# ootts/EasyHeC

Measured on AMD Instinct MI355X. Metric: mask-render fwd+bwd frames/sec, xArm7 50k-tri @1280x720x8-view, higher is better.
Workload: dtype f32; 1 GPU; xarm7_1280x720_8view; robot=xarm7 (41096 tris, 20525 verts), views_per_gpu=8, global_views=8, links=8, antialias=True, optimizer=Adam lr 3e-3 wd 5e-4, ref_sums=bound once, mask_output=False, step=HIP launch chain, parallelism=single GPU

## Files before the change

### easyhec_amd/_lib.py

```python
import ctypes
import os

_HERE = os.path.dirname(os.path.abspath(__file__))
LIB_PATH = os.environ.get("EHR_LIB") or os.path.join(_HERE, "libehr_hip.so")
_lib = None

c_void_p, c_int, c_size_t, c_float = ctypes.c_void_p, ctypes.c_int, ctypes.c_size_t, ctypes.c_float

SIGNATURES = {
    "ehr_version": (c_int, []),
    "ehr_last_error": (ctypes.c_char_p, []),
    "ehr_device_count": (c_int, []),
    "ehr_device_arch": (ctypes.c_char_p, [c_int]),
    "ehr_ctx_create": (c_int, [c_int, ctypes.POINTER(c_void_p)]),
    "ehr_ctx_destroy": (c_int, [c_void_p]),
    "ehr_ctx_scratch_bytes": (c_size_t, [c_void_p]),
    "ehr_tile_flags_bytes": (c_size_t, [c_int, c_int, c_int]),
    "ehr_rasterize_fwd": (c_int, [c_void_p, c_void_p, c_void_p, c_void_p, c_int, c_int, c_int, c_int, c_int, c_void_p,
                                  c_void_p, c_void_p, c_void_p]),
    "ehr_rasterize_grad": (c_int, [c_void_p, c_void_p, c_void_p, c_void_p, c_int, c_int, c_int, c_int, c_int, c_int,
                                   c_void_p, c_void_p, c_void_p]),
    "ehr_rasterize_grad_db": (c_int, [c_void_p, c_void_p, c_void_p, c_void_p, c_int, c_int, c_int, c_int, c_int, c_int,
                                   c_void_p, c_void_p]),
    "ehr_interpolate_fwd": (c_int, [c_void_p, c_void_p, c_void_p, c_int, c_int, c_int, c_int, c_int, c_int, c_int,
                                    c_void_p, c_void_p, c_void_p]),
    "ehr_interpolate_grad": (c_int, [c_void_p, c_void_p, c_void_p, c_void_p, c_int, c_int, c_int, c_int, c_int, c_int,
                                     c_int, c_void_p, c_void_p, c_void_p, c_void_p]),
    "ehr_interpolate_da_fwd": (c_int, [c_void_p, c_void_p, c_void_p, c_void_p, c_void_p] + [c_int] * 8 + [c_void_p, c_void_p]),
    "ehr_interpolate_da_grad": (c_int, [c_void_p, c_void_p, c_void_p, c_void_p, c_void_p, c_void_p] + [c_int] * 8 +
                                [c_void_p, c_void_p, c_void_p]),
    "ehr_topology_scratch_bytes": (c_size_t, [c_int]),
    "ehr_antialias_topology": (c_int, [c_void_p, c_int, c_void_p, c_void_p, c_size_t, c_void_p]),
    "ehr_antialias_work_bytes": (c_size_t, [c_int, c_int, c_int]),
    "ehr_antialias_fwd": (c_int, [c_void_p, c_void_p, c_void_p, c_void_p, c_void_p, c_int, c_int, c_int, c_int, c_int,
                                  c_int, c_int, c_void_p, c_void_p, c_void_p, c_void_p]),
    "ehr_antialias_fwd_zg": (c_int, [c_void_p, c_void_p, c_void_p, c_void_p, c_void_p, c_int, c_int, c_int, c_int, c_int,
                                     c_int, c_int, c_void_p, c_void_p, c_void_p, c_void_p, c_void_p]),
    "ehr_antialias_grad": (c_int, [c_void_p, c_void_p, c_void_p, c_void_p, c_void_p, c_void_p, c_int, c_int, c_int,
                                   c_int, c_int, c_int, c_int, c_void_p, c_void_p, c_void_p]),
    "ehr_fused_plan": (c_int, [c_void_p, c_int, c_int, c_int, c_int, c_int, c_int, c_float, c_void_p, c_void_p,
                                c_void_p, c_void_p]),
    "ehr_render_mask_loss": (c_int, [c_void_p, c_void_p, c_void_p, c_void_p, c_void_p, c_void_p, c_void_p, c_void_p,
                                     c_int, c_int, c_int, c_int, c_int, c_int, c_void_p, c_void_p, c_void_p,
                                     c_void_p]),
    "ehr_fused_status": (c_int, [c_void_p]),
    "ehr_fused_bind_ref": (c_int, [c_void_p, c_void_p, c_void_p]),
    "ehr_pose_forward": (c_int, [c_void_p, c_void_p, c_void_p, c_int, c_int, c_int, c_int, c_float, c_float, c_void_p,
                                 c_void_p, c_void_p, c_void_p, c_int, c_void_p]),
    "ehr_pose_backward": (c_int, [c_void_p, c_void_p, c_void_p, c_void_p, c_void_p, c_int, c_int, c_int, c_int,
                                  c_float, c_float, c_void_p, c_void_p]),
    "ehr_pose_adam": (c_int, [c_void_p, c_void_p, c_void_p, c_void_p, c_void_p, c_float, c_float, c_float, c_float,
                              c_float, c_void_p, c_void_p, c_void_p]),
    "ehr_solver_step": (c_int, [c_void_p] * 9 + [c_int] * 6 + [c_float] * 2 + [c_void_p] * 5 + [c_int, c_void_p] +
                        [c_float] * 5 + [c_void_p] * 8 + [c_int, c_void_p]),
    "ehr_solver_step_multi": (c_int, [c_void_p] * 9 + [c_int] * 7 + [c_float] * 2 + [c_void_p] * 5 + [c_int, c_void_p] +
                              [c_float] * 5 + [c_void_p] * 8 + [c_void_p]),
    "ehr_fused_bind_ref_shared": (c_int, [c_void_p, c_void_p, c_int, c_void_p]),
    "ehr_fused_bind_weight": (c_int, [c_void_p, c_void_p, c_int, c_void_p]),
    "ehr_mask_variance": (c_int, [c_void_p] * 5 + [c_int] * 7 + [c_void_p, c_void_p, c_int, c_void_p]),
    "ehr_mask_overlap": (c_int, [c_void_p] * 6 + [c_int] * 7 + [c_void_p, c_void_p, c_int, c_void_p]),
    "ehr_comm_unique_id": (c_int, [c_void_p]),
    "ehr_comm_init": (c_int, [c_void_p, c_void_p, c_int, c_int]),
    "ehr_comm_allreduce": (c_int, [c_void_p, c_void_p, c_int, c_void_p]),
    "ehr_comm_destroy": (c_int, [c_void_p]),
    "ehr_comm_p2p_export": (c_int, [c_void_p, c_void_p]),
    "ehr_comm_p2p_open": (c_int, [c_void_p, c_void_p, c_int, c_int]),
    "ehr_comm_p2p_step": (c_int, [c_void_p] * 6 + [c_float] * 5 + [c_void_p, c_void_p, c_void_p]),
    "ehr_comm_p2p_close": (c_int, [c_void_p]),
    "ehr_graph_begin": (c_int, [c_void_p, ctypes.POINTER(c_void_p)]),
    "ehr_graph_end": (c_int, [c_void_p]),
    "ehr_graph_launch": (c_int, [c_void_p, c_void_p]),
    "ehr_graph_release": (c_int, [c_void_p]),
    "ehr_fused_timing": (c_int, [c_void_p, c_int]),
    "ehr_fused_timing_read": (c_int, [c_void_p, ctypes.POINTER(c_float), ctypes.POINTER(c_int)]),
    "ehr_joint_forward": (c_int, [c_void_p] * 6 + [c_int] * 3 + [c_void_p, c_void_p, c_int, c_void_p, c_void_p, c_void_p]),
    "ehr_joint_backward_adam": (c_int, [c_void_p] * 3 + [c_int] * 5 + [c_float] * 2 + [c_void_p] * 10 + [c_float] * 5 +
                                [c_void_p, c_void_p]),
}


def lib():
    global _lib
    if _lib is None:
        if not os.path.exists(LIB_PATH):
            raise RuntimeError(
                f"{LIB_PATH} is missing: build it with `python -m easyhec_amd.build` (hipcc --offload-arch=gfx950). "
                "easyhec_amd has no CPU or PyTorch fallback for the render path.")
        l = ctypes.CDLL(LIB_PATH)
        for name, (res, args) in SIGNATURES.items():
            fn = getattr(l, name)
            fn.restype = res
            fn.argtypes = args
        _lib = l
    return _lib


def has_multistart():
    if not os.path.exists(LIB_PATH):
        return False
    return hasattr(_lib if _lib is not None else ctypes.CDLL(LIB_PATH), "ehr_solver_step_multi")


def has_pose_search():
    if not os.path.exists(LIB_PATH):
        return False
    return hasattr(_lib if _lib is not None else ctypes.CDLL(LIB_PATH), "ehr_mask_overlap")


def has_weighted_loss():
    if not os.path.exists(LIB_PATH):
        return False
    return hasattr(_lib if _lib is not None else ctypes.CDLL(LIB_PATH), "ehr_fused_bind_weight")


def has_joint_offsets():
    if not os.path.exists(LIB_PATH):
        return False
    l = _lib if _lib is not None else ctypes.CDLL(LIB_PATH)
    return hasattr(l, "ehr_joint_forward") and hasattr(l, "ehr_joint_backward_adam")


EHR_ERR_OVERFLOW = -3
EHR_ERR_RETRY = -4


def check(rc, what):
    if rc != 0:
        msg = lib().ehr_last_error().decode("utf-8", "replace")
        raise RuntimeError(f"{what}: {msg} (code {rc})")


def ptr(t):
    return None if t is None else c_void_p(t.data_ptr())
```

### easyhec_amd/csrc/ehr_device.h

```cpp
#pragma once
#include <hip/hip_runtime.h>
#include <stdint.h>

#define EHR_TILE_W 32
#define EHR_TILE_H 8
#define EHR_TILE_THREADS 256

namespace ehr {

typedef long long i64;
typedef unsigned long long u64;

__device__ __forceinline__ float tri_to_float(int x) {
    return (x <= 0x01000000) ? (float)x : __int_as_float(0x4a800000 + x);
}
__device__ __forceinline__ int float_to_tri(float f) {
    return (f <= 16777216.f) ? (int)f : (__float_as_int(f) - 0x4a800000);
}
__device__ __forceinline__ unsigned ord_key(float f) {
    unsigned u = __float_as_uint(f);
    return (u & 0x80000000u) ? ~u : (u | 0x80000000u);
}
__device__ __forceinline__ float ord_unkey(unsigned k) {
    unsigned u = (k & 0x80000000u) ? (k & 0x7fffffffu) : ~k;
    return __uint_as_float(u);
}
__device__ __forceinline__ float sat01(float x) { return x > 0.f ? (x < 1.f ? x : 1.f) : 0.f; }
__device__ __forceinline__ bool same_sign(float a, float b) {
    return (int)(__float_as_uint(a) ^ __float_as_uint(b)) >= 0;
}

__device__ __forceinline__ int snap_coord(float v, float w, float scale) {
    float s = v / w;
    float t = s * scale;
    t = fmaxf(fminf(t, 1073741824.f), -1073741824.f);
    return (int)rintf(t);
}

__device__ __forceinline__ float4 transform_vertex(const float* __restrict__ M, float x, float y, float z) {
    float4 o;
    o.x = fmaf(M[0], x, fmaf(M[1], y, fmaf(M[2], z, M[3])));
    o.y = fmaf(M[4], x, fmaf(M[5], y, fmaf(M[6], z, M[7])));
    o.z = fmaf(M[8], x, fmaf(M[9], y, fmaf(M[10], z, M[11])));
    o.w = fmaf(M[12], x, fmaf(M[13], y, fmaf(M[14], z, M[15])));
    return o;
}

struct ClipPoly {
    float4 q0, q1, q2, q3;
    int n;
};

__device__ __forceinline__ float4 clip_lerp(const float4& a, const float4& b, float da, float db) {
    float t = da / (da - db);
    float4 r;
    r.x = a.x + t * (b.x - a.x);
    r.y = a.y + t * (b.y - a.y);
    r.z = a.z + t * (b.z - a.z);
    r.w = a.w + t * (b.w - a.w);
    return r;
}

__device__ __forceinline__ ClipPoly clip_near_poly(const float4 p[3]) {
    ClipPoly c;
    c.n = 0;
    c.q0 = c.q1 = c.q2 = c.q3 = make_float4(0.f, 0.f, 0.f, 0.f);
    float d0 = p[0].z + p[0].w, d1 = p[1].z + p[1].w, d2 = p[2].z + p[2].w;
    bool all_in = (p[0].w > 0.f) && (p[1].w > 0.f) && (p[2].w > 0.f) && (d0 >= 0.f) && (d1 >= 0.f) && (d2 >= 0.f);
    if (all_in) {
        c.q0 = p[0];
        c.q1 = p[1];
        c.q2 = p[2];
        c.n = 3;
        return c;
    }
    const int mask = (d0 >= 0.f ? 1 : 0) | (d1 >= 0.f ? 2 : 0) | (d2 >= 0.f ? 4 : 0);
    const float4 I0 = clip_lerp(p[0], p[1], d0, d1);
    const float4 I1 = clip_lerp(p[1], p[2], d1, d2);
    const float4 I2 = clip_lerp(p[2], p[0], d2, d0);
    switch (mask) {
        case 1: c.q0 = p[0]; c.q1 = I0; c.q2 = I2; c.n = 3; break;
        case 2: c.q0 = I0; c.q1 = p[1]; c.q2 = I1; c.n = 3; break;
        case 4: c.q0 = I1; c.q1 = p[2]; c.q2 = I2; c.n = 3; break;
        case 3: c.q0 = p[0]; c.q1 = p[1]; c.q2 = I1; c.q3 = I2; c.n = 4; break;
        case 6: c.q0 = I0; c.q1 = p[1]; c.q2 = p[2]; c.q3 = I2; c.n = 4; break;
        case 5: c.q0 = p[0]; c.q1 = I0; c.q2 = I1; c.q3 = p[2]; c.n = 4; break;
        case 7: c.q0 = p[0]; c.q1 = p[1]; c.q2 = p[2]; c.n = 3; break;
        default: c.n = 0; break;
    }
    if (c.n < 3) c.n = 0;
    bool ok = (c.q0.w > 0.f) && (c.q1.w > 0.f) && (c.q2.w > 0.f) && (c.n < 4 || c.q3.w > 0.f);
    if (!ok) c.n = 0;
    return c;
}

struct Coverage {
    int X[3], Y[3];
    int ix0, ix1, iy0, iy1;
    bool valid;
};

__device__ __forceinline__ Coverage setup_coverage(const float4& a, const float4& b, const float4& c, int W, int H) {
    Coverage cv;
    const float sx = (float)(W * 8), sy = (float)(H * 8);
    cv.X[0] = snap_coord(a.x, a.w, sx);
    cv.Y[0] = snap_coord(a.y, a.w, sy);
    cv.X[1] = snap_coord(b.x, b.w, sx);
    cv.Y[1] = snap_coord(b.y, b.w, sy);
    cv.X[2] = snap_coord(c.x, c.w, sx);
    cv.Y[2] = snap_coord(c.y, c.w, sy);
    i64 area2 = (i64)(cv.X[1] - (i64)cv.X[0]) * (i64)(cv.Y[2] - (i64)cv.Y[0]) -
                (i64)(cv.X[2] - (i64)cv.X[0]) * (i64)(cv.Y[1] - (i64)cv.Y[0]);
    cv.valid = area2 != 0;
    if (area2 < 0) {
        int tx = cv.X[1], ty = cv.Y[1];
        cv.X[1] = cv.X[2];
        cv.Y[1] = cv.Y[2];
        cv.X[2] = tx;
        cv.Y[2] = ty;
    }
    int xmin = min(cv.X[0], min(cv.X[1], cv.X[2])), xmax = max(cv.X[0], max(cv.X[1], cv.X[2]));
    int ymin = min(cv.Y[0], min(cv.Y[1], cv.Y[2])), ymax = max(cv.Y[0], max(cv.Y[1], cv.Y[2]));
    const int cx = 8 - 8 * W, cy = 8 - 8 * H;
    int ix0 = (xmin - cx + 15) >> 4, ix1 = (xmax - cx) >> 4;
    int iy0 = (ymin - cy + 15) >> 4, iy1 = (ymax - cy) >> 4;
    ix0 = max(ix0, 0);
    iy0 = max(iy0, 0);
    ix1 = min(ix1, W - 1);
    iy1 = min(iy1, H - 1);
    cv.ix0 = ix0;
    cv.ix1 = ix1;
    cv.iy0 = iy0;
    cv.iy1 = iy1;
    if (ix0 > ix1 || iy0 > iy1) cv.valid = false;
    return cv;
}

struct EdgeEval {
    i64 e[3];
    i64 sx[3], sy[3];
};

__device__ __forceinline__ EdgeEval setup_edges(const Coverage& cv, int ix, int iy, int W, int H) {
    EdgeEval ee;
    const i64 cx = 8 - 8 * (i64)W, cy = 8 - 8 * (i64)H;
    i64 Px = 16 * (i64)ix + cx, Py = 16 * (i64)iy + cy;
#pragma unroll
    for (int k = 0; k < 3; k++) {
        int j = (k == 2) ? 0 : k + 1;
        i64 dX = (i64)cv.X[j] - cv.X[k], dY = (i64)cv.Y[j] - cv.Y[k];
        bool tl = (dY < 0) || (dY == 0 && dX < 0);
        ee.e[k] = dX * (Py - cv.Y[k]) - dY * (Px - cv.X[k]) - (tl ? 0 : 1);
        ee.sx[k] = -16 * dY;
        ee.sy[k] = 16 * dX;
    }
    return ee;
}

__device__ __forceinline__ void eval_pixel(const float4 p[3], float fx, float fy, float& a0, float& a1, float& a2) {
    float p0x = p[0].x - fx * p[0].w, p0y = p[0].y - fy * p[0].w;
    float p1x = p[1].x - fx * p[1].w, p1y = p[1].y - fy * p[1].w;
    float p2x = p[2].x - fx * p[2].w, p2y = p[2].y - fy * p[2].w;
    a0 = p1x * p2y - p1y * p2x;
    a1 = p2x * p0y - p2y * p0x;
    a2 = p0x * p1y - p0y * p1x;
}

__device__ __forceinline__ float eval_zw(const float4 p[3], float a0, float a1, float a2) {
    float z = (p[0].z * a0 + p[1].z * a1) + p[2].z * a2;
    float w = (p[0].w * a0 + p[1].w * a1) + p[2].w * a2;
    return z / w;
}


__device__ __forceinline__ bool rational_gt(float n0, float n1, float d0, float d1) {
    float l = n0 * d1, r = n1 * d0;
    bool flip = (d0 < 0.f) != (d1 < 0.f);
    return flip ? (l < r) : (l > r);
}

__device__ __forceinline__ int max_idx3(float n0, float n1, float n2, float d0, float d1, float d2) {
    bool g10 = rational_gt(n1, n0, d1, d0);
    bool g20 = rational_gt(n2, n0, d2, d0);
    bool g21 = rational_gt(n2, n1, d2, d1);
    if (g20 && g21) return 2;
    if (g10) return 1;
    return 0;
}

struct AAPair {
    bool found;
    int di;
    int tri1;
    float alpha;
};

__device__ __forceinline__ AAPair aa_analyze(const float4 p[3], const float4 o[3], int px, int py, int d, bool chose0,
                                             int W, int H) {
    AAPair r;
    r.found = false;
    r.di = 0;
    r.tri1 = chose0 ? 0 : 1;
    r.alpha = 0.f;
    float xh = .5f * (float)W, yh = .5f * (float)H;
    float w0 = 1.f / p[0].w, w1 = 1.f / p[1].w, w2 = 1.f / p[2].w;
    float ow0 = 1.f / o[0].w, ow1 = 1.f / o[1].w, ow2 = 1.f / o[2].w;
    float fx = (float)px + .5f - xh;
    float fy = (float)py + .5f - yh;
    float x0 = p[0].x * w0 * xh - fx, y0 = p[0].y * w0 * yh - fy;
    float x1 = p[1].x * w1 * xh - fx, y1 = p[1].y * w1 * yh - fy;
    float x2 = p[2].x * w2 * xh - fx, y2 = p[2].y * w2 * yh - fy;
    float ox0 = o[0].x * ow0 * xh - fx, oy0 = o[0].y * ow0 * yh - fy;
    float ox1 = o[1].x * ow1 * xh - fx, oy1 = o[1].y * ow1 * yh - fy;
    float ox2 = o[2].x * ow2 * xh - fx, oy2 = o[2].y * ow2 * yh - fy;

    float bb = (x1 - x0) * (y2 - y0) - (x2 - x0) * (y1 - y0);
    float a0 = (x1 - ox0) * (y2 - oy0) - (x2 - ox0) * (y1 - oy0);
    float a1 = (x2 - ox1) * (y0 - oy1) - (x0 - ox1) * (y2 - oy1);
    float a2 = (x0 - ox2) * (y1 - oy2) - (x1 - ox2) * (y0 - oy2);
    bool s0 = same_sign(a0, bb), s1 = same_sign(a1, bb), s2 = same_sign(a2, bb);
    if (!(s0 || s1 || s2)) return r;

    if (d) {
        float s;
        s = x0; x0 = y0; y0 = s;
        s = x1; x1 = y1; y1 = s;
        s = x2; x2 = y2; y2 = s;
    }
    float dx0 = x2 - x1, dx1 = x0 - x2, dx2 = x1 - x0;
    float dy0 = y2 - y1, dy1 = y0 - y2, dy2 = y1 - y0;
    const float F32_MAX = 3.402823466e+38f;
    float dc = -F32_MAX;
    float ds = chose0 ? 1.f : -1.f;
    float d0 = ds * (x1 * dy0 - y1 * dx0);
    float d1 = ds * (x2 * dy1 - y2 * dx1);
    float d2 = ds * (x0 * dy2 - y0 * dx2);
    if (same_sign(y1, y2)) { d0 = -F32_MAX; dy0 = 1.f; }
    if (same_sign(y2, y0)) { d1 = -F32_MAX; dy1 = 1.f; }
    if (same_sign(y0, y1)) { d2 = -F32_MAX; dy2 = 1.f; }
    int di = max_idx3(d0, d1, d2, dy0, dy1, dy2);
    if (di == 0 && s0 && fabsf(dy0) >= fabsf(dx0)) dc = d0 / dy0;
    if (di == 1 && s1 && fabsf(dy1) >= fabsf(dx1)) dc = d1 / dy1;
    if (di == 2 && s2 && fabsf(dy2) >= fabsf(dx2)) dc = d2 / dy2;
    const float eps = .0625f;
    if (dc > -eps && dc < 1.f + eps) {
        dc = fminf(fmaxf(dc, 0.f), 1.f);
        r.found = true;
        r.di = di;
        r.alpha = ds * (.5f - dc);
    }
    return r;
}

__device__ __forceinline__ void aa_pos_grad(float4 p1, float4 p2, int px, int py, int d, float alpha, float dd, int W,
                                            int H, float g1[3], float g2[3]) {
    float pxh = .5f * (float)W, pyh = .5f * (float)H;
    float fx = (float)px + .5f - pxh;
    float fy = (float)py + .5f - pyh;
    if (d) {
        float s;
        s = p1.x; p1.x = p1.y; p1.y = s;
        s = p2.x; p2.x = p2.y; p2.y = s;
        s = pxh; pxh = pyh; pyh = s;
        s = fx; fx = fy; fy = s;
    }
    float w1 = 1.f / p1.w, w2 = 1.f / p2.w;
    float x1 = p1.x * w1 * pxh - fx, y1 = p1.y * w1 * pyh - fy;
    float x2 = p2.x * w2 * pxh - fx, y2 = p2.y * w2 * pyh - fy;
    float dx = x2 - x1, dy = y2 - y1;
    float db = x1 * dy - y1 * dx;
    float ep = copysignf(1e-3f, dy);
    float iy = 1.f / (dy + ep);
    float dby = db * iy;
    float iw1 = -w1 * iy * dd;
    float iw2 = w2 * iy * dd;
    float gp1x = iw1 * pxh * y2;
    float gp2x = iw2 * pxh * y1;
    float gp1y = iw1 * pyh * (dby - x2);
    float gp2y = iw2 * pyh * (dby - x1);
    float gp1w = -(p1.x * gp1x + p1.y * gp1y) * w1;
    float gp2w = -(p2.x * gp2x + p2.y * gp2y) * w2;
    if (d) {
        float s;
        s = gp1x; gp1x = gp1y; gp1y = s;
        s = gp2x; gp2x = gp2y; gp2y = s;
    }
    if (fabsf(alpha) >= 0.5f) {
        gp1x = gp1y = gp1w = 0.f;
        gp2x = gp2y = gp2w = 0.f;
    }
    g1[0] = gp1x; g1[1] = gp1y; g1[2] = gp1w;
    g2[0] = gp2x; g2[1] = gp2y; g2[2] = gp2w;
}

constexpr int EHR_FLAG_TW = 32, EHR_FLAG_TH = 8;
__host__ __device__ __forceinline__ int flag_ntx(int W) { return (W + EHR_FLAG_TW - 1) / EHR_FLAG_TW; }
__host__ __device__ __forceinline__ int flag_nty(int H) { return (H + EHR_FLAG_TH - 1) / EHR_FLAG_TH; }
__device__ __forceinline__ bool tile_occupied(const unsigned char* __restrict__ flags, int b, int ix, int iy, int W, int H) {
    if (!flags) return true;
    const int ntx = flag_ntx(W), nty = flag_nty(H);
    return flags[((size_t)b * nty + (iy / EHR_FLAG_TH)) * ntx + (ix / EHR_FLAG_TW)] != 0;
}


__device__ __forceinline__ int lane_id() { return __lane_id(); }

template <int K>
__device__ __forceinline__ unsigned wave_xor_u32(unsigned v) {
    const int iv = (int)v;
    if (K == 1) return (unsigned)__builtin_amdgcn_update_dpp(iv, iv, 0xB1, 0xf, 0xf, false);
    if (K == 2) return (unsigned)__builtin_amdgcn_update_dpp(iv, iv, 0x4E, 0xf, 0xf, false);
    if (K == 4) {
        const int up = __builtin_amdgcn_update_dpp(iv, iv, 0x104, 0xf, 0xf, false);
        const int dn = __builtin_amdgcn_update_dpp(iv, iv, 0x114, 0xf, 0xf, false);
        return (unsigned)((__lane_id() & 4) ? dn : up);
    }
    if (K == 8) return (unsigned)__builtin_amdgcn_update_dpp(iv, iv, 0x128, 0xf, 0xf, false);
    if (K == 16) {
        const auto r = __builtin_amdgcn_permlane16_swap(v, v, false, false);
        return (__lane_id() & 16) ? r[0] : r[1];
    }
    const auto r = __builtin_amdgcn_permlane32_swap(v, v, false, false);
    return (__lane_id() & 32) ? r[0] : r[1];
}
template <int K>
__device__ __forceinline__ float wave_xor(float v) { return __uint_as_float(wave_xor_u32<K>(__float_as_uint(v))); }
template <int K>
__device__ __forceinline__ int wave_xor(int v) { return (int)wave_xor_u32<K>((unsigned)v); }
template <int K>
__device__ __forceinline__ long long wave_xor(long long v) {
    const unsigned long long u = (unsigned long long)v;
    const unsigned lo = wave_xor_u32<K>((unsigned)u), hi = wave_xor_u32<K>((unsigned)(u >> 32));
    return (long long)((unsigned long long)lo | ((unsigned long long)hi << 32));
}
template <int K>
__device__ __forceinline__ double wave_xor(double v) {
    const unsigned long long u = (unsigned long long)__double_as_longlong(v);
    const unsigned lo = wave_xor_u32<K>((unsigned)u), hi = wave_xor_u32<K>((unsigned)(u >> 32));
    return __longlong_as_double((long long)((unsigned long long)lo | ((unsigned long long)hi << 32)));
}

__device__ __forceinline__ float wave_sum(float v) {
    v += wave_xor<32>(v);
    v += wave_xor<16>(v);
    v += wave_xor<8>(v);
    v += wave_xor<4>(v);
    v += wave_xor<2>(v);
    v += wave_xor<1>(v);
    return v;
}

__device__ __forceinline__ int wave_sum12_element(int lane) {
    return 6 * ((lane >> 5) & 1) + 3 * ((lane >> 4) & 1) + ((lane & 8) ? 2 : ((lane >> 2) & 1));
}
__device__ __forceinline__ float wave_sum12(const float v[12], int lane) {
    const bool b32 = lane & 32, b16 = lane & 16, b8 = lane & 8, b4 = lane & 4;
    float a[6];
#pragma unroll
    for (int i = 0; i < 6; i++) {
        const float keep = b32 ? v[6 + i] : v[i], send = b32 ? v[i] : v[6 + i];
        a[i] = keep + wave_xor<32>(send);
    }
    float b[3];
#pragma unroll
    for (int i = 0; i < 3; i++) {
        const float keep = b16 ? a[3 + i] : a[i], send = b16 ? a[i] : a[3 + i];
        b[i] = keep + wave_xor<16>(send);
    }
    const float r0 = wave_xor<8>(b8 ? b[0] : b[2]);
    const float r1 = wave_xor<8>(b[1]);
    const float c0 = (b8 ? b[2] : b[0]) + r0, c1 = b[1] + r1;
    const float keep = b8 ? c0 : (b4 ? c1 : c0), send = b8 ? c0 : (b4 ? c0 : c1);
    float d = keep + wave_xor<4>(send);
    d += wave_xor<2>(d);
    d += wave_xor<1>(d);
    return d;
}

}
```

### easyhec_amd/csrc/ehr_fused.hip

```cpp
#include <stdlib.h>

#include <algorithm>

#include "ehr_fused_core.h"

namespace ehr {
constexpr int MAX_LINKS = 32;
}

using namespace ehr;

extern "C" {

int ehr_fused_plan(ehr_ctx* ctx, int B, int L, int V, int T, int H, int W, float slack, const float* verts,
                   const int32_t* tris, const int32_t* tri_link, const int32_t* opp) {
    if (!ctx) return fail(EHR_ERR_INVALID, "ehr_fused_plan: ctx is NULL");
    if (B <= 0 || L <= 0 || L > MAX_LINKS || V < 0 || T < 0 || H <= 0 || W <= 0 || H > 32768 || W > 32768)
        return fail(EHR_ERR_INVALID, "ehr_fused_plan: bad sizes (1 <= L <= %d)", MAX_LINKS);
    if (!(slack > 0.f)) slack = 0.f;
    if (ctx->gexec) {
        EHR_HIP(hipGraphExecDestroy(ctx->gexec));
        ctx->gexec = nullptr;
    }
    int rc0 = vbuf_plan(ctx, B, L, V, T, H, W, slack, verts, tris, tri_link, opp);
    if (rc0) return rc0;
    int dev = 0;
    EHR_HIP(hipGetDevice(&dev));
    hipDeviceProp_t prop;
    EHR_HIP(hipGetDeviceProperties(&prop, dev));
    ctx->num_cus = prop.multiProcessorCount;
    ctx->pB = B;
    ctx->pL = L;
    ctx->pV = V;
    ctx->pT = T;
    ctx->pH = H;
    ctx->pW = W;
    return EHR_OK;
}

static int fused_chain(ehr_ctx* ctx, const float* verts, const int32_t* tris, const int32_t* tri_link,
                       const int32_t* vert_link, const int32_t* opp, float* mvp, const float* ref, int B, int L, int V,
                       int T, int H, int W, float* mask, float* loss, float* grad_mvp, const StepHead* head,
                       const StepTail* tail, void* stream_, int multi_views = 0) {
    if (!ctx) return fail(EHR_ERR_INVALID, "fused op: ctx is NULL");
    if (!verts || !tris || !tri_link || !vert_link || !opp || !mvp || !ref || !loss)
        return fail(EHR_ERR_INVALID, "fused op: NULL tensor");
    if (ctx->pB != B || ctx->pL != L || ctx->pV != V || ctx->pT != T || ctx->pH != H || ctx->pW != W)
        return fail(EHR_ERR_INVALID, "fused op: shape differs from the planned one; call ehr_fused_plan first");
    return vbuf_chain(ctx, verts, tris, vert_link, opp, mvp, ref, B, L, V, T, H, W, mask, loss, grad_mvp, head,
                      tail, (hipStream_t)stream_, multi_views);
}

int ehr_render_mask_loss(ehr_ctx* ctx, const float* verts, const int32_t* tris, const int32_t* tri_link,
                         const int32_t* vert_link, const int32_t* opp, const float* mvp, const float* ref, int B,
                         int L, int V, int T, int H, int W, float* mask, float* loss, float* grad_mvp, void* stream) {
    return fused_chain(ctx, verts, tris, tri_link, vert_link, opp, const_cast<float*>(mvp), ref, B, L, V, T, H, W, mask,
                       loss, grad_mvp, nullptr, nullptr, stream);
}

static int step_head_tail(const char* who, ehr_ctx* ctx, ehr::Scratch ehr_ctx::*hstate, int nviews, int defer_adam,
                          int L, const float* K, const float* link_poses, float near_, float far_, float* dof, float* adam_m,
                          float* adam_v, int32_t* step, float* history, int history_rows, int32_t* history_row, float lr,
                          float beta1, float beta2, float eps, float weight_decay, float* tc_jac, const float* grad_mvp,
                          float* red, float* loss_out, float* grad_out, StepHead& head, StepTail& tail) {
    if (!ctx) return fail(EHR_ERR_INVALID, "%s: ctx is NULL", who);
    if (!K || !link_poses || !dof || !adam_m || !adam_v || !step || !tc_jac || !grad_mvp || !red)
        return fail(EHR_ERR_INVALID, "%s: NULL tensor", who);
    if (L > MAX_LINKS) return fail(EHR_ERR_INVALID, "%s: more than %d links", who, MAX_LINKS);
    if (history && !history_row) return fail(EHR_ERR_INVALID, "%s: history given without history_row", who);
    head.dof = dof;
    head.K = K;
    head.link_poses = link_poses;
    head.tc_jac = tc_jac;
    head.hist_row = history_row;
    head.history = history;
    head.history_rows = history_rows;
    head.n = near_;
    head.f = far_;
    head.adam_step = step;
    head.hstate = (int*)(ctx->*hstate).ptr;
    head.view0 = 0;
    head.nviews = nviews;
    tail.K = K;
    tail.link_poses = link_poses;
    tail.tc_jac = tc_jac;
    tail.red = red;
    tail.dof = dof;
    tail.m = adam_m;
    tail.v = adam_v;
    tail.step = step;
    tail.loss_out = loss_out;
    tail.grad_out = grad_out;
    tail.n = near_;
    tail.f = far_;
    tail.lr = lr;
    tail.b1 = beta1;
    tail.b2 = beta2;
    tail.eps = eps;
    tail.wd = weight_decay;
    tail.defer_adam = defer_adam;
    return EHR_OK;
}

int ehr_solver_step(ehr_ctx* ctx, const float* verts, const int32_t* tris, const int32_t* tri_link,
                    const int32_t* vert_link, const int32_t* opp, const float* K, const float* link_poses,
                    const float* ref, int B, int L, int V, int T, int H, int W, float near_, float far_, float* dof,
                    float* adam_m, float* adam_v, int32_t* step, float* history, int history_rows, int32_t* history_row,
                    float lr, float beta1,
                    float beta2, float eps, float weight_decay, float* mvp, float* tc_jac, float* mask, float* loss_b,
                    float* grad_mvp, float* red, float* loss_out, float* grad_out, int defer_adam, void* stream) {
    StepHead head;
    StepTail tail;
    int rc = step_head_tail("ehr_solver_step", ctx, &ehr_ctx::vb_hstate, B, defer_adam, L, K, link_poses, near_, far_, dof,
                            adam_m, adam_v, step, history, history_rows, history_row, lr, beta1, beta2, eps, weight_decay,
                            tc_jac, grad_mvp, red, loss_out, grad_out, head, tail);
    if (rc) return rc;
    return fused_chain(ctx, verts, tris, tri_link, vert_link, opp, mvp, ref, B, L, V, T, H, W, mask, loss_b, grad_mvp,
                       &head, &tail, stream);
}

int ehr_solver_step_multi(ehr_ctx* ctx, const float* verts, const int32_t* tris, const int32_t* tri_link,
                          const int32_t* vert_link, const int32_t* opp, const float* K, const float* link_poses,
                          const float* ref, int P, int Bv, int L, int V, int T, int H, int W, float near_, float far_,
                          float* dof, float* adam_m, float* adam_v, int32_t* step, float* history, int history_rows,
                          int32_t* history_row, float lr, float beta1, float beta2, float eps, float weight_decay,
                          float* mvp, float* tc_jac, float* mask, float* loss_b, float* grad_mvp, float* red,
                          float* loss_out, float* grad_out, void* stream) {
    StepHead head;
    StepTail tail;
    int rc = step_head_tail("ehr_solver_step_multi", ctx, &ehr_ctx::vb_hstate_m, Bv, 0, L, K, link_poses, near_, far_, dof,
                            adam_m, adam_v, step, history, history_rows, history_row, lr, beta1, beta2, eps, weight_decay,
                            tc_jac, grad_mvp, red, loss_out, grad_out, head, tail);
    if (rc) return rc;
    if (P <= 0 || Bv <= 0 || (long long)P * Bv > 0x7fffffffll / 64)
        return fail(EHR_ERR_INVALID, "ehr_solver_step_multi: bad P x Bv");
    if (ctx->pB != P * Bv || ctx->vb_hstate_m.cap < (size_t)VB_HSTATE_INTS * P * sizeof(int))
        return fail(EHR_ERR_INVALID, "ehr_solver_step_multi: call ehr_fused_plan for B = P x Bv = %d views first", P * Bv);
    return fused_chain(ctx, verts, tris, tri_link, vert_link, opp, mvp, ref, P * Bv, L, V, T, H, W, mask, loss_b, grad_mvp,
                       &head, &tail, stream, Bv);
}

int ehr_fused_bind_ref(ehr_ctx* ctx, const float* ref, void* stream) {
    return ehr_fused_bind_ref_shared(ctx, ref, ctx ? ctx->pB : 0, stream);
}

int ehr_fused_bind_ref_shared(ehr_ctx* ctx, const float* ref, int Bv, void* stream) {
    if (!ctx) return fail(EHR_ERR_INVALID, "ehr_fused_bind_ref: ctx is NULL");
    if (ctx->capturing) return fail(EHR_ERR_INVALID, "ehr_fused_bind_ref: not inside a graph capture");
    if (ctx->gexec) {
        EHR_HIP(hipGraphExecDestroy(ctx->gexec));
        ctx->gexec = nullptr;
    }
    if (!ref) {
        ctx->vb_ref = nullptr;
        return EHR_OK;
    }
    if (ctx->pB == 0) return fail(EHR_ERR_INVALID, "ehr_fused_bind_ref: call ehr_fused_plan first");
    return vbuf_bind_ref(ctx, ref, Bv, (hipStream_t)stream);
}

int ehr_fused_bind_weight(ehr_ctx* ctx, const float* weight, int Bv, void* stream) {
    (void)stream;
    if (!ctx) return fail(EHR_ERR_INVALID, "ehr_fused_bind_weight: ctx is NULL");
    if (ctx->capturing) return fail(EHR_ERR_INVALID, "ehr_fused_bind_weight: not inside a graph capture");
    if (weight) {
        if (ctx->pB == 0) return fail(EHR_ERR_INVALID, "ehr_fused_bind_weight: call ehr_fused_plan first");
        if (Bv <= 0 || ctx->pB % Bv != 0)
            return fail(EHR_ERR_INVALID, "ehr_fused_bind_weight: the plan's %d views are not a multiple of %d", ctx->pB, Bv);
    }
    if (ctx->gexec) {
        EHR_HIP(hipGraphExecDestroy(ctx->gexec));
        ctx->gexec = nullptr;
    }
    ctx->vb_ref = nullptr;
    ctx->vb_weight = weight;
    ctx->vb_weight_views = weight ? Bv : 0;
    return EHR_OK;
}

int ehr_fused_status(ehr_ctx* ctx) {
    if (!ctx) return fail(EHR_ERR_INVALID, "ehr_fused_status: ctx is NULL");
    if (ctx->pB == 0) return EHR_OK;
    if (!ctx->vb_acc.ptr) return EHR_OK;
    EHR_HIP(hipDeviceSynchronize());
    int m4[4] = {0, 0, 0, 0};
    int rc0 = vbuf_meta_read(ctx, m4);
    if (rc0) return rc0;
    if (m4[EHR_META_OVERFLOW] & VB_FLAG_NEED_SLOW) ctx->vb_slow_needed = true;
    if (m4[EHR_META_OVERFLOW] & ~VB_FLAG_NEED_SLOW)
        return fail(EHR_ERR_OVERFLOW, "fused path: an accumulator or the blended-pair spill pool overflowed");
    if (m4[EHR_META_OVERFLOW] & VB_FLAG_NEED_SLOW)
        return fail(EHR_ERR_RETRY, "fused path: the step met triangles for the general-triangle pass (near-plane clipping or "
                    "more than 512 pixels wide), which the solver step had not been launching; it is switched on now: run the "
                    "step again (its NaN left the optimiser state untouched; re-capture a captured chain)");
    return EHR_OK;
}


int ehr_graph_begin(ehr_ctx* ctx, void** capture_stream) {
    if (!ctx || !capture_stream) return fail(EHR_ERR_INVALID, "ehr_graph_begin: NULL argument");
    if (ctx->capturing) return fail(EHR_ERR_INVALID, "ehr_graph_begin: a capture is already open on this context");
    if (ctx->timing) return fail(EHR_ERR_INVALID, "ehr_graph_begin: disable ehr_fused_timing first");
    if (!ctx->cap_stream) EHR_HIP(hipStreamCreateWithFlags(&ctx->cap_stream, hipStreamNonBlocking));
    if (ctx->gexec) {
        EHR_HIP(hipGraphExecDestroy(ctx->gexec));
        ctx->gexec = nullptr;
    }
    EHR_HIP(hipStreamBeginCapture(ctx->cap_stream, hipStreamCaptureModeThreadLocal));
    ctx->capturing = true;
    *capture_stream = (void*)ctx->cap_stream;
    return EHR_OK;
}

int ehr_graph_end(ehr_ctx* ctx) {
    if (!ctx || !ctx->capturing) return fail(EHR_ERR_INVALID, "ehr_graph_end: no open capture");
    ctx->capturing = false;
    hipGraph_t graph = nullptr;
    EHR_HIP(hipStreamEndCapture(ctx->cap_stream, &graph));
    if (!graph) return fail(EHR_ERR_HIP, "ehr_graph_end: the capture was invalidated");
    hipError_t e = hipGraphInstantiate(&ctx->gexec, graph, nullptr, nullptr, 0);
    (void)hipGraphDestroy(graph);
    if (e != hipSuccess) {
        ctx->gexec = nullptr;
        return fail(EHR_ERR_HIP, "hipGraphInstantiate failed: %s", hipGetErrorString(e));
    }
    ctx->gexec_reallocs = ctx->scratch_moves();
    return EHR_OK;
}

int ehr_graph_launch(ehr_ctx* ctx, void* stream) {
    if (!ctx || !ctx->gexec) return fail(EHR_ERR_INVALID, "ehr_graph_launch: no instantiated graph");
    if (ctx->gexec_reallocs != ctx->scratch_moves())
        return fail(EHR_ERR_INVALID, "ehr_graph_launch: library scratch was reallocated after the capture; capture again");
    EHR_HIP(hipGraphLaunch(ctx->gexec, (hipStream_t)stream));
    return EHR_OK;
}

int ehr_graph_release(ehr_ctx* ctx) {
    if (!ctx) return EHR_OK;
    if (ctx->capturing) {
        hipGraph_t graph = nullptr;
        (void)hipStreamEndCapture(ctx->cap_stream, &graph);
        if (graph) (void)hipGraphDestroy(graph);
        ctx->capturing = false;
    }
    if (ctx->gexec) {
        EHR_HIP(hipGraphExecDestroy(ctx->gexec));
        ctx->gexec = nullptr;
    }
    return EHR_OK;
}

int ehr_fused_timing(ehr_ctx* ctx, int enable) {
    if (!ctx) return fail(EHR_ERR_INVALID, "ehr_fused_timing: ctx is NULL");
    ctx->timing = enable != 0;
    ctx->ev_used = 0;
    return EHR_OK;
}

int ehr_fused_timing_read(ehr_ctx* ctx, float* ms, int* ncalls) {
    if (!ctx || !ms || !ncalls) return fail(EHR_ERR_INVALID, "ehr_fused_timing_read: NULL argument");
    EHR_HIP(hipDeviceSynchronize());
    const size_t per = EHR_FUSED_STAGES + 1;
    const size_t n = ctx->ev_used / per;
    for (int s = 0; s < EHR_FUSED_STAGES; s++) ms[s] = 0.f;
    for (size_t c = 0; c < n; c++)
        for (int s = 0; s < EHR_FUSED_STAGES; s++) {
            float t = 0.f;
            EHR_HIP(hipEventElapsedTime(&t, ctx->ev[c * per + s], ctx->ev[c * per + s + 1]));
            ms[s] += t;
        }
    *ncalls = (int)n;
    ctx->ev_used = 0;
    return EHR_OK;
}

}
```

### easyhec_amd/csrc/ehr_host.h

```cpp
#pragma once
#include <hip/hip_runtime.h>
#include <stdint.h>
#include <stdio.h>

#include <string>
#include <vector>

#include "../../include/ehr.h"

struct ehr_ctx;

namespace ehr {

void set_error(const std::string& msg);
int fail(int code, const char* fmt, ...);

#define EHR_HIP(call)                                                                                   \
    do {                                                                                                \
        hipError_t e_ = (call);                                                                         \
        if (e_ != hipSuccess)                                                                           \
            return ::ehr::fail(EHR_ERR_HIP, "%s failed: %s (%s:%d)", #call, hipGetErrorString(e_), __FILE__, __LINE__); \
    } while (0)

#define EHR_LAUNCH_CHECK()                                                                              \
    do {                                                                                                \
        hipError_t e_ = hipGetLastError();                                                              \
        if (e_ != hipSuccess)                                                                           \
            return ::ehr::fail(EHR_ERR_HIP, "kernel launch failed: %s (%s:%d)", hipGetErrorString(e_), __FILE__, __LINE__); \
    } while (0)

struct Scratch {
    void* ptr = nullptr;
    size_t cap = 0;
    int reserve(size_t bytes);
    void release();
    unsigned long long moves = 0;
    bool pinned = false;
};

int zero_words(void* dst, size_t nwords, hipStream_t stream);
int fill_words(void* dst, size_t nwords, unsigned value, hipStream_t stream);
int copy_words(void* dst, const void* src, size_t nwords, hipStream_t stream);

struct StepHead;
struct StepTail;
struct RasterShape {
    int B, V, T, H, W, ranged;
    bool operator==(const RasterShape& o) const { return B == o.B && V == o.V && T == o.T && H == o.H && W == o.W && ranged == o.ranged; }
};
#define VB_LOSS_SLOTS 32
#define VB_LOSS_STRIDE 16
#define VB_FLAG_NEED_SLOW 4
#define VB_MAX_UNITS 512
#define VB_SPILL_ITEMS (1 << 20)
int vbuf_plan(ehr_ctx* ctx, int B, int L, int V, int T, int H, int W, float slack, const float* verts,
              const int32_t* tris, const int32_t* tri_link, const int32_t* opp);
int vbuf_meta_read(ehr_ctx* ctx, int* meta4);
int vbuf_bind_ref(ehr_ctx* ctx, const float* ref, int views, hipStream_t stream);
int vbuf_score(ehr_ctx* ctx, const float* verts, const int32_t* tris, const int32_t* vert_link, const float* mvp, int Q, int S,
               int L, int V, int T, int H, int W, long long* score, unsigned char* count, hipStream_t stream, int* handled);
int vbuf_overlap(ehr_ctx* ctx, const float* verts, const int32_t* tris, const int32_t* vert_link, const float* mvp,
                 const float* ref, int Q, int S, int L, int V, int T, int H, int W, long long* overlap, long long* ref_area,
                 hipStream_t stream, int* handled);
int vbuf_chain(ehr_ctx* ctx, const float* verts, const int32_t* tris, const int32_t* vert_link,
               const int32_t* opp, float* mvp, const float* ref, int B, int L, int V, int T, int H, int W, float* mask,
               float* loss, float* grad_mvp, const StepHead* head, const StepTail* tail, hipStream_t stream,
               int multi_views = 0);

}

struct ehr_ctx {
    int device = 0;
    ehr::Scratch counts;
    unsigned long long counts_clean = ~0ull;
    bool vb_slow_needed = false;
    ehr::Scratch ranges;
    std::vector<int32_t> ranges_last;
    unsigned long long ranges_moves = ~0ull;
    ehr::Scratch rkeys;
    unsigned long long rkeys_clean = ~0ull;
    ehr::Scratch offsets;
    ehr::Scratch entries;
    size_t entries_cap = 0;
    int* host_pinned = nullptr;
    hipEvent_t ev_size[2] = {nullptr, nullptr};
    bool size_valid[2] = {false, false};
    ehr::RasterShape size_shape[2] = {};
    int size_slot = 0;
    int pB = 0, pL = 0, pV = 0, pT = 0, pH = 0, pW = 0;
    int num_cus = 256;
    ehr::Scratch vb_clus;
    ehr::Scratch vb_heavy;
    ehr::Scratch vb_idx;
    const void* vb_plan_tris = nullptr;
    const void* vb_plan_opp = nullptr;
    const void* vb_plan_verts = nullptr;
    int vb_nc = 0;
    int vb_jcap = 0;
    int vb_chunk = 0;
    ehr::Scratch vb_boxes;
    ehr::Scratch vb_units;
    ehr::Scratch vb_acc;
    ehr::Scratch vb_posc;
    bool vb_lazy = false;
    ehr::Scratch vb_jobs;
    ehr::Scratch vb_spill;
    int vb_spill_cap = 0;
    ehr::Scratch vb_refsum;
    const float* vb_ref = nullptr;
    int vb_ref_views = 0;
    const float* vb_weight = nullptr;
    int vb_weight_views = 0;
    ehr::Scratch vb_hstate;
    ehr::Scratch vb_hstate_m;
    ehr::Scratch sc_counts, sc_offsets, sc_entries, sc_posc;
    ehr::Scratch sc_img;
    size_t sc_entries_cap = 0;
    ehr::Scratch sc_clus, sc_misc;
    int sc_nc = 0;
    const void* sc_key[3] = {nullptr, nullptr, nullptr};
    int sc_key_n[3] = {0, 0, 0};
    unsigned long long sc_hash = 0;
    bool sc_mixed = false;
    void* comm = nullptr;
    int comm_ranks = 0;
    void* p2p_mail = nullptr;
    void* p2p_peer[EHR_P2P_MAX_RANKS] = {};
    int p2p_ranks = 0, p2p_rank = 0;
    hipStream_t cap_stream = nullptr;
    hipGraphExec_t gexec = nullptr;
    unsigned long long gexec_reallocs = 0;
    unsigned long long scratch_moves() const {
        unsigned long long n = 0;
        for (const ehr::Scratch* s : {&counts, &offsets, &entries, &vb_clus, &vb_heavy, &vb_idx, &vb_boxes, &vb_units, &vb_acc,
                                      &vb_posc, &vb_jobs, &vb_spill, &vb_refsum, &vb_hstate, &vb_hstate_m, &sc_counts, &sc_offsets, &sc_entries, &sc_posc, &sc_clus, &sc_misc, &sc_img})
            n += s->moves;
        return n;
    }
    bool capturing = false;
    bool timing = false;
    std::vector<hipEvent_t> ev;
    size_t ev_used = 0;
};
```

### easyhec_amd/csrc/ehr_vbuf.hip

```cpp
#include <stdlib.h>
#include <string.h>

#include <algorithm>
#include <utility>
#include <vector>

#include "ehr_fused_core.h"

namespace ehr {

constexpr int VB_RW = EHR_TILE_W + 2;
constexpr int VB_RH = EHR_TILE_H + 2;
constexpr int VB_RN = VB_RW * VB_RH;
constexpr int VB_WORDS = (VB_RN + 63) / 64;
constexpr int VB_LBOX_STRIDE = 16;
constexpr int VB_HEAVY_T_DEFAULT = 3000;
constexpr int VB_HEAVY_CAP = 4096;
constexpr int VB_MED_CAP = 2048;
constexpr int VB_MED_T_DEFAULT = 1500;
constexpr int VB_PRIO_LONG = 3;
constexpr int VB_PRIO_HEAVY = 2;
constexpr int VB_JOB_ITEMS = 64;
constexpr int VB_SPILL_BLOCK = 2048;
constexpr u64 VB_EMPTY = ~0ull;
constexpr int VB_VERTEX_GRID = 5;
constexpr int VB_JOB_GRID = 4;
constexpr int VB_COMPOSITE_GRID = 6;
constexpr int VB_SCORE_COUNT_GRID = 4;
constexpr int VB_SLOW_GRID = 32;
constexpr bool VB_XCD_SPLIT = true;
constexpr int VB_FAST_EXTENT = 8192;

constexpr int VB_XCDS = 8;
constexpr int VB_XCD_BITS = __builtin_ctz(VB_XCDS);
static_assert(VB_XCDS == 1 << VB_XCD_BITS, "a workgroup finds its XCD with a mask and a shift");
__host__ __device__ constexpr int vb_xcd_share(int n) { return (n + VB_XCDS - 1) >> VB_XCD_BITS; }
__host__ __device__ constexpr int vb_xcd_round_up(int n) { return (n + VB_XCDS - 1) & ~(VB_XCDS - 1); }

enum VbLine {
    VB_LINE_JOB_CURSOR = 0,
    VB_LINE_COMP_ARRIVE = VB_LINE_JOB_CURSOR + VB_XCDS,
    VB_LINE_SLOW_COUNT = VB_LINE_COMP_ARRIVE + VB_XCDS,
    VB_LINES
};
__host__ __device__ __forceinline__ int* vb_line(int* meta, int k) {
    return (int*)((((uintptr_t)(meta + EHR_META_INTS)) + 127) & ~(uintptr_t)127) + 32 * k;
}
constexpr size_t VB_META_BYTES = EHR_META_INTS * sizeof(int) + (VB_LINES + 1) * 128;

#define VB_WAVE_SYNC() asm volatile("s_waitcnt lgkmcnt(0)" ::: "memory")

struct VbItem {
    int packed;
    int v1, v2;
    float alpha;
};

struct VbCarve {
    uintptr_t at;
    template <class T>
    T* take(size_t n, size_t align = alignof(T)) {
        at = (at + align - 1) & ~(uintptr_t)(align - 1);
        T* const p = (T*)at;
        at += n * sizeof(T);
        return p;
    }
};

struct VbSlots {
    float* jval;
    VbItem* jitems;
    int* jn;
    int* jspill;
    int* jbase;
    unsigned* jutile;
    int4* slow_list;
    int jcap;
};
constexpr size_t VB_SLOT_BYTES = 256 * sizeof(float) + VB_JOB_ITEMS * sizeof(VbItem) + 2 * sizeof(int) + sizeof(int4);
static_assert(VB_SLOT_BYTES == 1024 + 1024 + 8 + 16, "job slot: 2072 bytes");
static VbSlots vb_slots(void* base, size_t jcap, size_t units, size_t* bytes = nullptr) {
    VbCarve c{(uintptr_t)base};
    VbSlots s;
    s.jval = c.take<float>(jcap * 256);
    s.jitems = c.take<VbItem>(jcap * VB_JOB_ITEMS);
    s.jn = c.take<int>(jcap);
    s.jspill = c.take<int>(jcap);
    s.jbase = c.take<int>(units + 1);
    s.jutile = c.take<unsigned>(units);
    s.slow_list = c.take<int4>(jcap, 16);
    s.jcap = (int)jcap;
    if (bytes) *bytes = c.at - (uintptr_t)base;
    return s;
}

constexpr bool vb_interior(int i) {
    return (i % VB_RW) >= 1 && (i % VB_RW) <= EHR_TILE_W && (i / VB_RW) >= 1 && (i / VB_RW) <= EHR_TILE_H;
}
constexpr u64 vb_word_h(int k) {
    u64 w = 0;
    for (int j = 0; j < 64; j++) {
        const int i = 64 * k + j;
        if (i + 1 < VB_RN && (i % VB_RW) != VB_RW - 1 && (vb_interior(i) || vb_interior(i + 1))) w |= 1ull << j;
    }
    return w;
}
constexpr u64 vb_word_v(int k) {
    u64 w = 0;
    for (int j = 0; j < 64; j++) {
        const int i = 64 * k + j;
        if (i + VB_RW < VB_RN && (vb_interior(i) || vb_interior(i + VB_RW))) w |= 1ull << j;
    }
    return w;
}

template <int S>
__device__ __forceinline__ void vb_shr(const u64 in[VB_WORDS], u64 out[VB_WORDS]) {
#pragma unroll
    for (int k = 0; k < VB_WORDS; k++) out[k] = (in[k] >> S) | (k + 1 < VB_WORDS ? in[k + 1] << (64 - S) : 0ull);
}

__device__ __forceinline__ int vb_readlane(int v, int lane) { return __builtin_amdgcn_readlane(v, lane); }
__device__ __forceinline__ float vb_readlane(float v, int lane) {
    return __int_as_float(__builtin_amdgcn_readlane(__float_as_int(v), lane));
}
__device__ __forceinline__ float4 vb_readlane(const float4& v, int lane) {
    return make_float4(vb_readlane(v.x, lane), vb_readlane(v.y, lane), vb_readlane(v.z, lane), vb_readlane(v.w, lane));
}
__device__ __forceinline__ int vb_mbcnt(u64 m) {
    return __builtin_amdgcn_mbcnt_hi((unsigned)(m >> 32), __builtin_amdgcn_mbcnt_lo((unsigned)m, 0u));
}


struct VbHeavy {
    int* gen;
    int* list;
    int* mlist;
    int* stamp;
    int mcap;
    int heavy_base;
    int heavy_max;
};

static VbHeavy vb_heavy(void* base, size_t nstamp, size_t* bytes = nullptr) {
    VbCarve c{(uintptr_t)base};
    VbHeavy hv = {};
    hv.gen = c.take<int>(8);
    hv.list = c.take<int>(2 * VB_HEAVY_CAP);
    hv.mlist = c.take<int>(2 * VB_MED_CAP);
    hv.stamp = c.take<int>(nstamp);
    if (bytes) *bytes = c.at - (uintptr_t)base;
    return hv;
}

__device__ __forceinline__ int vb_hint_pack(int u, int tx, int ty) { return tx | (ty << 10) | (u << 22); }
__device__ __forceinline__ int vb_hint_dense(int id, int nt, int ntx) {
    return (int)((unsigned)id >> 22) * nt + ((id >> 10) & 4095) * ntx + (id & 1023);
}
static_assert(VB_MAX_UNITS <= 1024, "vb_hint_pack");
struct VbClusters {
    const int32_t* ctri;
    const int32_t* clink;
    const int32_t* coff;
    const float* laabb;
    const float4* cvert;
    int NC;
};

__device__ __forceinline__ uint2 vb_pack_box(int x0, int y0, int x1, int y1) {
    return make_uint2((unsigned)x0 | ((unsigned)y0 << 16), (unsigned)x1 | ((unsigned)y1 << 16));
}
#define VB_BOX_EMPTY make_uint2(0xffffffffu, 0u)

struct VbEdges {
    int e0, e1, e2, sx0, sx1, sx2, sy0, sy1, sy2;
};
__device__ __forceinline__ VbEdges vb_edges(int X0, int Y0, int X1, int Y1, int X2, int Y2, int bx0, int by0, int W,
                                            int H) {
    VbEdges r;
    const int ox = 16 * bx0 + 8 - 8 * W, oy = 16 * by0 + 8 - 8 * H;
    X0 -= ox; X1 -= ox; X2 -= ox;
    Y0 -= oy; Y1 -= oy; Y2 -= oy;
    {
        const int dX = X1 - X0, dY = Y1 - Y0;
        r.e0 = __mul24(dX, 0 - Y0) - __mul24(dY, 0 - X0) - (((dY < 0) || (dY == 0 && dX < 0)) ? 0 : 1);
        r.sx0 = -16 * dY;
        r.sy0 = 16 * dX;
    }
    {
        const int dX = X2 - X1, dY = Y2 - Y1;
        r.e1 = __mul24(dX, 0 - Y1) - __mul24(dY, 0 - X1) - (((dY < 0) || (dY == 0 && dX < 0)) ? 0 : 1);
        r.sx1 = -16 * dY;
        r.sy1 = 16 * dX;
    }
    {
        const int dX = X0 - X2, dY = Y0 - Y2;
        r.e2 = __mul24(dX, 0 - Y2) - __mul24(dY, 0 - X2) - (((dY < 0) || (dY == 0 && dX < 0)) ? 0 : 1);
        r.sx2 = -16 * dY;
        r.sy2 = 16 * dX;
    }
    return r;
}

struct VbRecs {
    uint2* tbox;
    uint2* cbox;
    int4* trec;
    size_t n;
};
constexpr size_t VB_REC_BYTES = sizeof(int4) * 2 + sizeof(uint2);
constexpr size_t VB_CLUSTER_REC_BYTES = 64 * VB_REC_BYTES + sizeof(uint2);
static_assert(VB_CLUSTER_REC_BYTES == 2568, "raster records: 64 x (32 + 8) + 8 bytes per (view, cluster)");
static VbRecs vb_recs(void* base, size_t views, size_t NC, size_t* bytes = nullptr) {
    VbCarve c{(uintptr_t)base};
    VbRecs r;
    r.n = views * NC * 64;
    r.trec = c.take<int4>(r.n * 2);
    r.tbox = c.take<uint2>(r.n);
    r.cbox = c.take<uint2>(views * NC);
    if (bytes) *bytes = c.at - (uintptr_t)base;
    return r;
}

__device__ __forceinline__ bool vb_depth_safe(const float4& p0, const float4& p1, const float4& p2, int W, int H, bool pos = false) {
    const float r0 = __builtin_amdgcn_rcpf(p0.w), r1 = __builtin_amdgcn_rcpf(p1.w), r2 = __builtin_amdgcn_rcpf(p2.w);
    const float z0 = p0.z * r0, z1 = p1.z * r1, z2 = p2.z * r2;
    const float sx = (float)(8 * W), sy = (float)(8 * H);
    const float x0 = p0.x * r0 * sx, y0 = p0.y * r0 * sy;
    const float d1x = p1.x * r1 * sx - x0, d1y = p1.y * r1 * sy - y0;
    const float d2x = p2.x * r2 * sx - x0, d2y = p2.y * r2 * sy - y0;
    const float q1 = fabsf(z1 - z0), q2 = fabsf(z2 - z0);
    const float A = fabsf(d1x * d2y - d2x * d1y);
    const float l1 = fabsf(d1x) + fabsf(d1y), l2 = fabsf(d2x) + fabsf(d2y);
    const float delta = 0.66f * (q1 * l2 + q2 * l1) * __builtin_amdgcn_rcpf(A) + 0.275f * (q1 + q2);
    const float zmax = fmaxf(z0, fmaxf(z1, z2)), zmin = fminf(z0, fminf(z1, z2));
    const float wmax = fmaxf(p0.w, fmaxf(p1.w, p2.w)), wmin = fminf(p0.w, fminf(p1.w, p2.w));
    return (A >= 0.055f * (l1 + l2) + 1.1e-3f) && (wmax <= 4.f * wmin) && (zmax + delta <= 1.f - 1.1e-5f) &&
           (zmin - delta >= (pos ? 1.1e-5f : -1.f + 1.1e-5f));
}

typedef unsigned short vb_u16x2 __attribute__((ext_vector_type(2)));
__device__ __forceinline__ unsigned vb_pk_min_u16(unsigned a, unsigned b) {
    return __builtin_bit_cast(unsigned, __builtin_elementwise_min(__builtin_bit_cast(vb_u16x2, a), __builtin_bit_cast(vb_u16x2, b)));
}
__device__ __forceinline__ unsigned vb_pk_max_u16(unsigned a, unsigned b) {
    return __builtin_bit_cast(unsigned, __builtin_elementwise_max(__builtin_bit_cast(vb_u16x2, a), __builtin_bit_cast(vb_u16x2, b)));
}

constexpr int VB_SMALL_BOX = 3;
constexpr int VB_VERTEX_WAVES = 5;
enum VbRole {
    VB_ROLE_FIRST_CHUNK = 1,
    VB_ROLE_LATER_CHUNK = 2,
    VB_ROLE_CHUNK_MASK = 3,
    VB_ROLE_POS_ONLY = 4,
};
template <bool HEAD, bool MULTI = false>
__global__ void __launch_bounds__(256, VB_VERTEX_WAVES)
vb_vertex_kernel(const float* __restrict__ verts, const int32_t* __restrict__ vert_link,
                 const int32_t* __restrict__ tris, VbClusters cl, StepHead head, float* __restrict__ mvp, int V, int nvb,
                 BinGeom g, float4* __restrict__ posc, VbRecs rc, int* __restrict__ lbox, int* __restrict__ zacc,
                 int nzacc, int* __restrict__ meta, int B, int gx, int xcd_views, VbHeavy hv, int chunk_role) {
    __shared__ float Tc[16];
    __shared__ float M[32][16];
    int b, bx;
    if (xcd_views > 0) {
        const int xcd = blockIdx.x & (VB_XCDS - 1), k = blockIdx.x >> VB_XCD_BITS;
        b = xcd * xcd_views + k / gx;
        bx = k - (k / gx) * gx;
    } else {
        b = blockIdx.x / gx;
        bx = blockIdx.x - b * gx;
    }
    const int tid = threadIdx.x, L = g.L, H = g.H, W = g.W;
    const bool pos_only = (chunk_role & VB_ROLE_POS_ONLY) != 0;
    chunk_role &= VB_ROLE_CHUNK_MASK;
    const bool first = bx == 0 && b == 0 && chunk_role == VB_ROLE_FIRST_CHUNK;
    const bool rearm = bx == 0 && b == 0 && chunk_role == VB_ROLE_LATER_CHUNK;
    int hyp = 0, bview = b;
    if (MULTI) {
        const int bg = head.view0 + b;
        hyp = bg / head.nviews;
        bview = bg - hyp * head.nviews;
        head.dof += 6 * hyp;
    }
    const bool first_head = MULTI ? (bx == 0 && bview == 0) : first;
    const int nitems = nvb + (cl.NC + 3) / 4;
    const int lane = tid & 63;
    int item = bx;
    int l = -1, t = -1;
    float vx[3] = {0.f, 0.f, 0.f}, vy[3] = {0.f, 0.f, 0.f}, vz[3] = {0.f, 0.f, 0.f};
    bool have = false;
    auto load_geometry = [&](int it) {
        l = -1;
        t = -1;
        have = false;
        if (it < nvb) {
            const int v = it * 256 + tid;
            if (v < V) {
                l = vert_link[v];
                vx[0] = verts[3 * v];
                vy[0] = verts[3 * v + 1];
                vz[0] = verts[3 * v + 2];
                have = true;
            }
        } else {
            const int c = (it - nvb) * 4 + (tid >> 6);
            if (c < cl.NC) {
                const size_t cs = (size_t)c * 64 + lane, cn = (size_t)cl.NC * 64;
                t = cl.ctri[cs];
                l = cl.clink[c];
                const float4 q0 = cl.cvert[cs], q1 = cl.cvert[cn + cs], q2 = cl.cvert[2 * cn + cs];
                vx[0] = q0.x; vy[0] = q0.y; vz[0] = q0.z;
                vx[1] = q0.w; vy[1] = q1.x; vz[1] = q1.y;
                vx[2] = q1.z; vy[2] = q1.w; vz[2] = q2.x;
                have = t >= 0 && q2.y != 0.f;
            }
        }
    };
    if (item < nitems) load_geometry(item);
    __shared__ int lacc[32][4];
    if (tid < 128) lacc[tid >> 2][tid & 3] = (tid & 2) ? -1 : INT_MAX;
    __shared__ float LP[32][16];
    __shared__ float Kc[9];
    float dofv[6] = {0.f, 0.f, 0.f, 0.f, 0.f, 0.f};
    if (HEAD) {
#pragma unroll
        for (int k = 0; k < 6; k++) dofv[k] = head.dof[k];
        float lpv[2] = {0.f, 0.f};
        float kv = 0.f;
#pragma unroll
        for (int j = 0; j < 2; j++)
            if (tid + 256 * j < L * 16) lpv[j] = head.link_poses[(size_t)bview * L * 16 + tid + 256 * j];
        if (tid >= 64 && tid < 73) kv = head.K[tid - 64];
#pragma unroll
        for (int j = 0; j < 2; j++)
            if (tid + 256 * j < L * 16) LP[(tid + 256 * j) >> 4][(tid + 256 * j) & 15] = lpv[j];
        if (tid >= 64 && tid < 73) Kc[tid - 64] = kv;
    }
    if (HEAD && tid < 6) {
        Dual<1> T6[16];
        se3_exp_dual<1>(dofv, 1e-4f, T6, tid);
        if (tid == 0)
            for (int i = 0; i < 16; i++) Tc[i] = T6[i].v;
        if (first_head) {
            if (MULTI) {
                head.tc_jac += 7 * 16 * hyp;
                if (head.history && head.hist_row) {
                    head.hist_row += hyp;
                    head.history += (size_t)hyp * head.history_rows * 6;
                }
                head.adam_step += hyp;
                head.hstate += VB_HSTATE_INTS * hyp;
            }
            for (int i = 0; i < 16; i++) {
                if (tid == 0) head.tc_jac[i] = T6[i].v;
                head.tc_jac[16 * (tid + 1) + i] = T6[i].d[0];
            }
            if (tid == 0 && head.history && head.hist_row) {
                int row = head.hist_row[0];
                if (head.hstate && head.adam_step) {
                    const int t1 = head.adam_step[0] + 1;
                    if (head.hstate[0] == t1 && head.hstate[1] && head.hstate[2] == row && row > 0) row -= 1;
                    head.hstate[0] = t1;
                }
                const bool adv = row >= 0 && row < head.history_rows;
                if (adv) {
                    for (int k = 0; k < 6; k++) head.history[6 * row + k] = dofv[k];
                    head.hist_row[0] = row + 1;
                }
                if (head.hstate) {
                    head.hstate[1] = adv ? 1 : 0;
                    head.hstate[2] = adv ? row + 1 : row;
                }
            }
        }
    }
    if (first) {
        __shared__ int s_gen;
        if (tid == 0) {
            s_gen = hv.gen[0] + 1;
            hv.gen[0] = s_gen;
            hv.gen[1 + (s_gen & 1)] = 0;
            hv.gen[4 + (s_gen & 1)] = 0;
            {
                const int nprev = hv.gen[1 + ((s_gen - 1) & 1)];
                int thr = max(hv.gen[6], hv.heavy_base);
                if (nprev > hv.heavy_max)
                    thr = min(thr + (thr >> 3), 1 << 24);
                else if (2 * nprev < hv.heavy_max)
                    thr = max(hv.heavy_base, thr - (thr >> 4));
                hv.gen[6] = thr;
            }
        }
        __syncthreads();
        {
            const int gen = s_gen, cur = (gen - 1) & 1;
            const int n = min(hv.gen[1 + cur], VB_HEAVY_CAP);
            for (int i = tid; i < n; i += 256) hv.stamp[min(vb_hint_dense(hv.list[cur * VB_HEAVY_CAP + i], g.nt, g.ntx), B * L * g.nt - 1)] = gen;
            const int n2 = min(hv.gen[4 + cur], hv.mcap);
            for (int i = tid; i < n2; i += 256) hv.stamp[min(vb_hint_dense(hv.mlist[cur * VB_MED_CAP + i], g.nt, g.ntx), B * L * g.nt - 1)] = -gen;
        }
        if (tid < 8) meta[tid] = 0;
        if (tid < VB_LINES) *vb_line(meta, tid) = 0;
    }
    if (rearm) {
        if (tid < 8 && tid != EHR_META_OVERFLOW) meta[tid] = 0;
        if (tid < VB_LINES) *vb_line(meta, tid) = 0;
    }
    if (bx == 0) {
        const int nzv = nzacc / B;
        for (int i = tid; i < nzv; i += 256) zacc[(size_t)b * nzv + i] = 0;
    }
    __syncthreads();
    if (HEAD) {
        if (tid < L) {
            float P[16], C[16];
            projection(Kc, H, W, head.n, head.f, P);
            mvp_from_pose(Tc, P, LP[tid], C);
            for (int k = 0; k < 16; k++) M[tid][k] = C[k];
            if (bx == 0)
                for (int k = 0; k < 16; k++) mvp[((size_t)b * L + tid) * 16 + k] = C[k];
        }
    } else {
        for (int i = tid; i < L * 16; i += 256) M[i >> 4][i & 15] = mvp[(size_t)b * L * 16 + i];
    }
    __syncthreads();
    for (; item < nitems;) {
    const bool lv = (unsigned)l < (unsigned)L;
    if (item < nvb) {
        const int v = item * 256 + tid;
        if (v < V) {
            float4 o = make_float4(0.f, 0.f, 0.f, -1.f);
            if (lv) o = transform_vertex(M[l], vx[0], vy[0], vz[0]);
            posc[(size_t)b * V + v] = o;
        }
    } else {
    const int c = (item - nvb) * 4 + (tid >> 6);
    const bool cvalid = c < cl.NC;
    int x0 = 0xffff, y0 = 0xffff, x1 = 0, y1 = 0;
    int4 r0 = make_int4(-1, -1, -1, 0), r1 = make_int4(0, 0, t, 0);
    if (have && lv) {
        const float4 p0 = transform_vertex(M[l], vx[0], vy[0], vz[0]);
        const float4 p1 = transform_vertex(M[l], vx[1], vy[1], vz[1]);
        const float4 p2 = transform_vertex(M[l], vx[2], vy[2], vz[2]);
        const bool simple = (p0.w > 0.f) && (p1.w > 0.f) && (p2.w > 0.f) && (p0.z + p0.w >= 0.f) &&
                            (p1.z + p1.w >= 0.f) && (p2.z + p2.w >= 0.f);
        if (!simple) {
            const float4 pp[3] = {p0, p1, p2};
            const ClipPoly cp = clip_near_poly(pp);
            for (int sidx = 0; sidx + 2 < cp.n; sidx++) {
                const Coverage cv = (sidx == 0) ? setup_coverage(cp.q0, cp.q1, cp.q2, W, H) : setup_coverage(cp.q0, cp.q2, cp.q3, W, H);
                if (!cv.valid) continue;
                const int ax = max(cv.ix0, 0), ay = max(cv.iy0, 0), bx1 = min(cv.ix1, W - 1), by1 = min(cv.iy1, H - 1);
                if (ax > bx1 || ay > by1) continue;
                x0 = min(x0, ax);
                y0 = min(y0, ay);
                x1 = max(x1, bx1);
                y1 = max(y1, by1);
            }
            r1.w = 1;
        } else {
            const Coverage cv = setup_coverage(p0, p1, p2, W, H);
            if (cv.valid) {
                x0 = cv.ix0; y0 = cv.iy0; x1 = cv.ix1; y1 = cv.iy1;
                const unsigned ex = (unsigned)max(cv.X[0], max(cv.X[1], cv.X[2])) - (unsigned)min(cv.X[0], min(cv.X[1], cv.X[2]));
                const unsigned ey = (unsigned)max(cv.Y[0], max(cv.Y[1], cv.Y[2])) - (unsigned)min(cv.Y[0], min(cv.Y[1], cv.Y[2]));
                if (ex > VB_FAST_EXTENT || ey > VB_FAST_EXTENT) {
                    r1.w = 1;
                } else {
                    const VbEdges ed = vb_edges(cv.X[0], cv.Y[0], cv.X[1], cv.Y[1], cv.X[2], cv.Y[2], x0, y0, W, H);
                    if (x1 - x0 < VB_SMALL_BOX && y1 - y0 < VB_SMALL_BOX) {
                        const int bw = x1 - x0 + 1, bh = y1 - y0 + 1;
                        bool any = false;
                        int q0 = ed.e0, q1 = ed.e1, q2 = ed.e2;
#pragma unroll
                        for (int j = 0; j < VB_SMALL_BOX; j++) {
                            int a0 = q0, a1 = q1, a2 = q2;
#pragma unroll
                            for (int i = 0; i < VB_SMALL_BOX; i++) {
                                any = any || (i < bw && j < bh && (a0 | a1 | a2) >= 0);
                                a0 += ed.sx0;
                                a1 += ed.sx1;
                                a2 += ed.sx2;
                            }
                            q0 += ed.sy0;
                            q1 += ed.sy1;
                            q2 += ed.sy2;
                        }
                        if (!any) {
                            x0 = 0xffff; y0 = 0xffff; x1 = 0; y1 = 0;
                        }
                    }
                    r0 = make_int4(ed.e0, ed.e1, ed.e2, (int)(((unsigned)(ed.sy0 / 16) & 0xffffu) | ((unsigned)(-ed.sx0 / 16) << 16)));
                    r1.x = (int)(((unsigned)(ed.sy1 / 16) & 0xffffu) | ((unsigned)(-ed.sx1 / 16) << 16));
                    r1.y = (int)(((unsigned)(ed.sy2 / 16) & 0xffffu) | ((unsigned)(-ed.sx2 / 16) << 16));
                    r1.w = vb_depth_safe(p0, p1, p2, W, H, pos_only) ? 0 : 2;
                }
            }
        }
    }
    const size_t slot = ((size_t)b * cl.NC + (cvalid ? c : 0)) * 64 + lane;
    if (cvalid) rc.tbox[slot] = vb_pack_box(x0, y0, x1, y1);
    if (cvalid && x0 <= x1) {
        rc.trec[2 * slot] = r0;
        rc.trec[2 * slot + 1] = r1;
    }
    const uint2 pbox = vb_pack_box(x0, y0, x1, y1);
    unsigned bmin = pbox.x, bmax = pbox.y;
#define VB_BOX_STEP(ctrl, rows)                                                                       \
    bmin = vb_pk_min_u16(bmin, (unsigned)__builtin_amdgcn_update_dpp((int)bmin, (int)bmin, ctrl, rows, 0xf, false)); \
    bmax = vb_pk_max_u16(bmax, (unsigned)__builtin_amdgcn_update_dpp((int)bmax, (int)bmax, ctrl, rows, 0xf, false));
    VB_BOX_STEP(0x111, 0xf) VB_BOX_STEP(0x112, 0xf) VB_BOX_STEP(0x114, 0xf) VB_BOX_STEP(0x118, 0xf)
    VB_BOX_STEP(0x142, 0xa) VB_BOX_STEP(0x143, 0xc)
#undef VB_BOX_STEP
    const int a = (int)(bmin & 0xffffu), bq = (int)(bmin >> 16), cc = (int)(bmax & 0xffffu), d = (int)(bmax >> 16);
    if (lane == 63) {
        const bool cne = cvalid && a <= cc;
        if (cvalid) rc.cbox[(size_t)b * cl.NC + c] = cne ? vb_pack_box(a, bq, cc, d) : VB_BOX_EMPTY;
        if (cne && lv) {
            atomicMin(&lacc[l][0], a);
            atomicMin(&lacc[l][1], bq);
            atomicMax(&lacc[l][2], cc);
            atomicMax(&lacc[l][3], d);
        }
    }
    }
    item += gx;
    if (item < nitems) load_geometry(item);
    }
    __syncthreads();
    if (tid < 4 * L && lacc[tid >> 2][0] != INT_MAX) {
        int* const lb = lbox + VB_LBOX_STRIDE * ((size_t)b * L + (tid >> 2));
        if (tid & 2)
            atomicMax(lb + (tid & 3), lacc[tid >> 2][tid & 3]);
        else
            atomicMin(lb + (tid & 3), lacc[tid >> 2][tid & 3]);
    }
}


__device__ __forceinline__ int vb_div_rw(int i) { return (int)(__umul24((unsigned)i, 1928u) >> 16); }
static_assert(VB_RW == 34, "vb_div_rw");
#define VB_DPP_(v, ctrl, rows) __builtin_amdgcn_update_dpp(0, (v), (ctrl), (rows), 0xf, false)
__device__ __forceinline__ int vb_scan_add(int v) {
    v += VB_DPP_(v, 0x111, 0xf);
    v += VB_DPP_(v, 0x112, 0xf);
    v += VB_DPP_(v, 0x114, 0xf);
    v += VB_DPP_(v, 0x118, 0xf);
    v += VB_DPP_(v, 0x142, 0xa);
    v += VB_DPP_(v, 0x143, 0xc);
    return v;
}
__device__ __forceinline__ int vb_scan_max(int v) {
    v = max(v, VB_DPP_(v, 0x111, 0xf));
    v = max(v, VB_DPP_(v, 0x112, 0xf));
    v = max(v, VB_DPP_(v, 0x114, 0xf));
    v = max(v, VB_DPP_(v, 0x118, 0xf));
    v = max(v, VB_DPP_(v, 0x142, 0xa));
    v = max(v, VB_DPP_(v, 0x143, 0xc));
    return v;
}
__device__ __forceinline__ int vb_div_small(int x, float inv) { return (int)(((float)x + 0.5f) * inv); }
__device__ __forceinline__ int vb_next_set(u64 m, int j) { return j + __ffsll((unsigned long long)(m >> (j + 1))); }

struct VbRegion {
    int x0, y0, x1, y1;
};

struct VbLazy {
    const float* verts;
    const float* M;
    const float4* pc;
};
template <bool LAZY>
struct VbVertsT;
template <>
struct VbVertsT<true> {
    const float* verts;
    float M[16];
    __device__ __forceinline__ float4 operator[](int v) const {
        const float* a = verts + 3 * (size_t)v;
        return transform_vertex(M, a[0], a[1], a[2]);
    }
};
template <>
struct VbVertsT<false> {
    const float4* pc;
    __device__ __forceinline__ float4 operator[](int v) const { return pc[v]; }
};
template <bool LAZY>
__device__ __forceinline__ VbVertsT<LAZY> vb_verts(const VbLazy& z);
template <>
__device__ __forceinline__ VbVertsT<true> vb_verts<true>(const VbLazy& z) {
    VbVertsT<true> r;
    r.verts = z.verts;
#pragma unroll
    for (int k = 0; k < 16; k++) r.M[k] = __int_as_float(__builtin_amdgcn_readfirstlane(__float_as_int(z.M[k])));
    return r;
}
template <>
__device__ __forceinline__ VbVertsT<false> vb_verts<false>(const VbLazy& z) {
    VbVertsT<false> r;
    r.pc = z.pc;
    return r;
}

#define VB_SPAN_GW 4
constexpr int VB_DL = 640;
constexpr int VB_SQ = 256;
constexpr unsigned VB_ID_COVERED = 0xfffffffeu;
constexpr u64 VB_ROW_MASK = (1ull << VB_RW) - 1ull;

struct alignas(16) VbRaster {
    int e[64][3];
    unsigned dxy[64][3];
    unsigned box[64];
    unsigned ent[64];
    int pre[65];
};
struct alignas(16) VbWaveLds {
    u64 key[VB_RN];
    u64 cov[VB_RH];
    u64 need[VB_RH];
    u64 intr[VB_RH];
    u64 intr_and[3][VB_RH];
    VbRaster R;
    unsigned dl[VB_DL];
    unsigned sq[VB_SQ];
    int bad;
};

__device__ __forceinline__ bool vb_depth_test(const float4 p[3], int t, int ix, int iy, int W, int H, u64* slot,
                                              bool* nonpos = nullptr) {
    const float xs = 2.f / (float)W, xo = 1.f / (float)W - 1.f;
    const float ys = 2.f / (float)H, yo = 1.f / (float)H - 1.f;
    const float fx = (float)ix * xs + xo;
    const float fy = (float)iy * ys + yo;
    float a0, a1, a2;
    eval_pixel(p, fx, fy, a0, a1, a2);
    const float zw = eval_zw(p, a0, a1, a2);
    if (zw >= -1.f && zw <= 1.f) {
        if (nonpos) {
            if (!(zw > 0.f)) *nonpos = true;
        } else {
            atomicMin(slot, ((u64)ord_key(zw) << 32) | (unsigned)t);
        }
        return true;
    }
    return false;
}

struct VbSlotIdx {
    const int4* cvidx;
};

__device__ __forceinline__ void vb_raster_wide(float4 pa, float4 pb, float4 pc, int t, int W, int H, VbRegion rg, int rx0,
                                            int ry0, u64* key, u64* cov) {
    const int lane = lane_id();
    const float4 p[3] = {pa, pb, pc};
    const ClipPoly c = clip_near_poly(p);
    for (int s = 0; s + 2 < c.n; s++) {
        Coverage cv = (s == 0) ? setup_coverage(c.q0, c.q1, c.q2, W, H) : setup_coverage(c.q0, c.q2, c.q3, W, H);
        if (!cv.valid) continue;
        const int bx0 = max(cv.ix0, rg.x0), by0 = max(cv.iy0, rg.y0);
        const int bx1 = min(cv.ix1, rg.x1), by1 = min(cv.iy1, rg.y1);
        if (bx0 > bx1 || by0 > by1) continue;
        const int bw = bx1 - bx0 + 1, npx = bw * (by1 - by0 + 1);
        const EdgeEval ee = setup_edges(cv, bx0, by0, W, H);
        for (int i0 = 0; i0 < npx; i0 += 64) {
            const int i = i0 + lane;
            if (i < npx) {
                const int dy = i / bw, dx = i - dy * bw;
                const i64 e0 = ee.e[0] + dx * ee.sx[0] + dy * ee.sy[0];
                const i64 e1 = ee.e[1] + dx * ee.sx[1] + dy * ee.sy[1];
                const i64 e2 = ee.e[2] + dx * ee.sx[2] + dy * ee.sy[2];
                if ((e0 | e1 | e2) >= 0) {
                    const int ix = bx0 + dx, iy = by0 + dy;
                    if (vb_depth_test(p, t, ix, iy, W, H, &key[(iy - ry0) * VB_RW + (ix - rx0)]))
                        atomicOr((unsigned long long*)&cov[iy - ry0], 1ull << (ix - rx0));
                }
            }
        }
    }
}

template <bool COVER = false, bool LAZY = false>
__device__ __forceinline__ void vb_flush(VbWaveLds& S, u64* key, u64* cov, int n, const VbLazy& pvz,
                                      const int4* __restrict__ cvidx_link, int W, int H, int rx0, int ry0) {
    const int lane = lane_id();
    VB_WAVE_SYNC();
    if (lane < VB_RH) {
        const u64 c = cov[lane];
        const u64 up = (lane + 1 < VB_RH) ? cov[lane + 1] : VB_ROW_MASK;
        const u64 dn = (lane > 0) ? cov[lane - 1] : VB_ROW_MASK;
        const u64 inner = ((c >> 1) | (1ull << (VB_RW - 1))) & ((c << 1) | 1ull) & up & dn;
        S.need[lane] = c & ~inner & VB_ROW_MASK;
    }
    VB_WAVE_SYNC();
    int nk = 0;
    for (int base = 0; base < n; base += 64) {
        const int i = base + lane;
        unsigned e = 0;
        bool keep = false;
        if (i < n) {
            e = S.dl[i];
            const int pix = e & 511u, row = vb_div_rw(pix), col = pix - row * VB_RW;
            const unsigned m4 = (e >> 9) & 15u;
            const unsigned m = (e & (1u << 13)) ? m4 : (m4 & (unsigned)(S.need[row] >> col));
            keep = m != 0;
            e = (e & ~(15u << 9)) | (m << 9);
        }
        const u64 km = __ballot(keep);
        if (keep) S.dl[nk + vb_mbcnt(km)] = e;
        nk += __popcll(km);
    }
    VB_WAVE_SYNC();
    const VbVertsT<LAZY> pv = vb_verts<LAZY>(pvz);
    for (int base = 0; base < nk; base += 64) {
        const int i = base + lane;
        if (i < nk) {
            const unsigned e = S.dl[i];
            const int4 vi = cvidx_link[e >> 14];
            const float4 p[3] = {pv[vi.x], pv[vi.y], pv[vi.z]};
            const int pix = e & 511u, row = vb_div_rw(pix), col = pix - row * VB_RW;
            const unsigned m = (e >> 9) & 15u;
            const bool flag = (e >> 13) & 1u;
            unsigned drawn = 0, mm = m;
            while (mm) {
                const int k = __ffs(mm) - 1;
                mm &= mm - 1;
                bool nonpos = false;
                if (vb_depth_test(p, vi.w, rx0 + col + k, ry0 + row, W, H, &key[pix + k], COVER ? &nonpos : nullptr)) drawn |= 1u << k;
                if (COVER && nonpos) S.bad = 1;
            }
            if (flag && drawn) atomicOr((unsigned long long*)&cov[row], (u64)drawn << col);
        }
    }
    VB_WAVE_SYNC();
}

template <bool WIDE, bool COVER = false, bool LAZY = false>
__device__ __forceinline__ int vb_raster_round(bool sv, size_t slot, unsigned srel, const VbRecs& rc, const VbRegion& rg,
                                               int rx0, int ry0, int W, int H, VbWaveLds& S, u64* key, u64* cov, int n,
                                               const VbLazy& pv, const int4* __restrict__ cvidx_link, bool& full,
                                               int& cost, int qh) {
    VbRaster& R = S.R;
    const int lane = lane_id();
    int units = 0, srows = 0;
    bool wide = false;
    uint2 bx = VB_BOX_EMPTY;
    int4 r0 = make_int4(0, 0, 0, 0), r1 = r0;
    if (sv) {
        bx = rc.tbox[slot];
        r0 = rc.trec[2 * slot];
        r1 = rc.trec[2 * slot + 1];
    }
    bool has_in = false;
    {
        u64 in = 0;
        if (lane < VB_RH) {
            const u64 c = cov[lane];
            const u64 up = (lane + 1 < VB_RH) ? cov[lane + 1] : VB_ROW_MASK;
            const u64 dn = (lane > 0) ? cov[lane - 1] : VB_ROW_MASK;
            in = COVER ? (c & VB_ROW_MASK) : (c & ((c >> 1) | (1ull << (VB_RW - 1))) & ((c << 1) | 1ull) & up & dn & VB_ROW_MASK);
            S.intr[lane] = in;
// ... 1417 lines not shown
}
__device__ __forceinline__ VbWeight vb_comp_weight(VbCompParamsWPtr p) {
    VbWeight wt;
    wt.w = p->wt.w;
    wt.view0 = p->wt.view0;
    wt.nviews = p->wt.nviews;
    return wt;
}
typedef const VbCompParams __attribute__((address_space(4)))* VbCompParamsPtr;
__device__ __forceinline__ VbCompParamsPtr vb_comp_params() {
    VbCompParamsPtr p = (VbCompParamsPtr)__builtin_amdgcn_kernarg_segment_ptr();
    asm volatile("" : "+s"(p));
    return p;
}

constexpr int VB_FINISH_POLLS = 1 << 21;
__device__ __forceinline__ int vb_comp_arrivals(int xcd, int per, int nitems, int nfill, int nlbox) {
    const int share = vb_xcd_share(nitems);
    const int mine = max(0, min(share, nitems - xcd * share));
    int n = (mine + 3) >> 2;
    const int fwg = (nfill + 3) >> 2, lwg = (nlbox + 255) >> 8;
    n = max(n, fwg > xcd ? vb_xcd_share(fwg - xcd) : 0);
    n = max(n, lwg > xcd ? vb_xcd_share(lwg - xcd) : 0);
    return min(n, per);
}

template <bool TAIL, bool FILL, bool SHARED = false, bool WEIGHTED = false>
__global__ void __launch_bounds__(256, FILL ? 5 : 6)
vb_composite_kernel(VbCompArgs C, StepTail tail, VbSharedRef sh, VbWeight wt) {
    __shared__ float gpix_all[4][EHR_TILE_W * EHR_TILE_H];
    extern __shared__ int s_dyn[];
    const int tid = threadIdx.x, lane = tid & 63, wave = tid >> 6;
    float* const gpix = gpix_all[wave];
    const int U = C.B * C.g.L;
    int* const s_jbase = s_dyn;
    unsigned* const s_utile = reinterpret_cast<unsigned*>(s_dyn + U + 1);
    const bool sparse = C.tsum != nullptr;
    for (int i = tid; i <= U; i += 256) s_jbase[i] = C.sl.jbase[i];
    for (int i = tid; i < U; i += 256) s_utile[i] = C.sl.jutile[i];
    if (C.do_finish && C.lbox_all)
        for (int i = (int)blockIdx.x * 256 + tid; i < VB_LBOX_STRIDE * C.B_all * C.g.L; i += (int)gridDim.x * 256)
            C.lbox_all[i] = (i & 2) ? INT_MIN : INT_MAX;
    __syncthreads();
    const int nwg = gridDim.x, xcd = blockIdx.x & (VB_XCDS - 1);
    vb_composite_items<FILL, SHARED, WEIGHTED>(C, s_jbase, s_utile, gpix, xcd, (int)(blockIdx.x >> VB_XCD_BITS) * 4 + wave, (nwg >> VB_XCD_BITS) * 4, nwg, sh);
    if (!vb_comp_params()->C.do_finish) return;
    const VbCompParamsPtr Q = vb_comp_params();
    const int per = nwg >> VB_XCD_BITS;
    const int nitems = sparse ? min(s_jbase[U], Q->C.sl.jcap) : Q->C.B * Q->C.g.nt;
    const int nfill = FILL ? Q->C.B * Q->C.g.nt : 0, nlbox = Q->C.lbox_all ? VB_LBOX_STRIDE * Q->C.B_all * Q->C.g.L : 0;
    const int kblk = (int)(blockIdx.x >> VB_XCD_BITS);
    const bool finisher = (int)blockIdx.x == nwg - VB_XCDS;
    const bool arrives = kblk < vb_comp_arrivals(xcd, per, nitems, nfill, nlbox);
    if (!finisher) {
        if (!arrives) return;
        asm volatile("s_waitcnt vmcnt(0)" ::: "memory");
        __syncthreads();
        if (tid == 0)
            (void)__hip_atomic_fetch_add(vb_line(Q->C.meta, VB_LINE_COMP_ARRIVE + xcd), 1, __ATOMIC_RELAXED, __HIP_MEMORY_SCOPE_AGENT);
        return;
    }
    __shared__ double S[4][17];
    __shared__ float red_lds[8];
    __shared__ float Js[6][16];
    const long long* const vtot = sparse ? Q->C.vtot_all : nullptr;
    const BinGeom g = ((const VbCompParams*)Q)->C.g;
    const StepTail tl = ((const VbCompParams*)Q)->tail;
    FinishPre pre;
    __syncthreads();
    finish_prefetch<TAIL>(pre, g, Q->C.B_all, vtot, tl, Q->C.nls, Js, gpix_all[0]);
    if (Q->C.ref_flag && tid == 0 && Q->C.ref_flag[0]) atomicOr(&Q->C.meta[EHR_META_OVERFLOW], 1);
    if (wave == 0) {
        int* const ctr = vb_line(Q->C.meta, VB_LINE_COMP_ARRIVE + (lane & (VB_XCDS - 1)));
        const int want = vb_comp_arrivals(lane & (VB_XCDS - 1), per, nitems, nfill, nlbox) - (((lane & (VB_XCDS - 1)) == 0 && arrives) ? 1 : 0);
        bool done = false;
        for (int polls = 0; polls < VB_FINISH_POLLS; polls++) {
            const int have = (lane < VB_XCDS) ? __hip_atomic_load(ctr, __ATOMIC_RELAXED, __HIP_MEMORY_SCOPE_AGENT) : want;
            done = __ballot(have < want) == 0;
            if (done) break;
            __builtin_amdgcn_s_sleep(2);
        }
        if (lane < VB_XCDS) __hip_atomic_store(ctr, 0, __ATOMIC_RELAXED, __HIP_MEMORY_SCOPE_AGENT);
        if (!done && lane == 0) atomicOr(&Q->C.meta[EHR_META_OVERFLOW], 1);
    }
    asm volatile("s_waitcnt vmcnt(0)" ::: "memory");
    __syncthreads();
    __builtin_amdgcn_fence(__ATOMIC_ACQUIRE, "agent");
    finish_reduce<TAIL>(pre, g, Q->C.B_all, Q->C.facc_all, vtot, Q->C.loss, Q->C.grad_mvp, Q->C.meta, tl, Q->C.nls, VB_LOSS_STRIDE, S, red_lds, Js, gpix_all[0]);
}

__global__ void __launch_bounds__(256)
vb_finish_multi_kernel(MultiFinish A, StepTail tail) {
    __shared__ double S[4][17];
    __shared__ float red_lds[8];
    __shared__ float Js[6][16];
    __shared__ float lp_lds[1024];
    const int p = blockIdx.x, tid = threadIdx.x, L = A.g.L;
    for (int i = p * 256 + tid; i < VB_LBOX_STRIDE * A.P * A.Bv * L; i += (int)gridDim.x * 256)
        A.lbox_all[i] = (i & 2) ? INT_MIN : INT_MAX;
    tail.tc_jac += 7 * 16 * p;
    tail.red += 8 * p;
    tail.dof += 6 * p;
    tail.m += 6 * p;
    tail.v += 6 * p;
    tail.step += p;
    if (tail.loss_out) tail.loss_out += p;
    if (tail.grad_out) tail.grad_out += 6 * p;
    const size_t v0 = (size_t)p * A.Bv;
    const long long* const vtot = A.vtot_all ? A.vtot_all + v0 : nullptr;
    FinishPre pre;
    finish_prefetch<true>(pre, A.g, A.Bv, vtot, tail, A.nls, Js, lp_lds);
    if (A.ref_flag && tid == 0 && A.ref_flag[0]) atomicOr(&A.meta[EHR_META_OVERFLOW], 1);
    __syncthreads();
    finish_reduce<true>(pre, A.g, A.Bv, A.facc_all + v0 * vb_acc_stride(L, A.nls), vtot, A.loss + v0,
                        A.grad_mvp + v0 * L * 16, A.meta, tail, A.nls, VB_LOSS_STRIDE, S, red_lds, Js, lp_lds);
}

__global__ void __launch_bounds__(256)
vb_hash_kernel(const unsigned* __restrict__ a, size_t na, const unsigned* __restrict__ b, size_t nb, const unsigned* __restrict__ c,
               size_t nc, unsigned long long* __restrict__ out) {
    unsigned long long h = 0;
    const size_t n = na + nb + nc;
    for (size_t i = (size_t)blockIdx.x * 256 + threadIdx.x; i < n; i += (size_t)gridDim.x * 256) {
        const unsigned w = i < na ? a[i] : (i < na + nb ? b[i - na] : c[i - na - nb]);
        unsigned long long x = (unsigned long long)w + 0x9e3779b97f4a7c15ull * ((unsigned long long)i + 1ull);
        x ^= x >> 33;
        x *= 0xff51afd7ed558ccdull;
        x ^= x >> 33;
        x *= 0xc4ceb9fe1a85ec53ull;
        x ^= x >> 33;
        h += x;
    }
#pragma unroll
    for (int o = 32; o > 0; o >>= 1) h += __shfl_xor(h, o, 64);
    if ((threadIdx.x & 63) == 0) atomicAdd(out, h);
}

__global__ void __launch_bounds__(256)
vb_score_count_kernel(BinGeom g, int nq, int S, const u64* __restrict__ tcov, unsigned long long* __restrict__ sacc,
                      unsigned char* __restrict__ count_img, int* __restrict__ lbox, int nlbox,
                      unsigned long long* __restrict__ prev_sacc, long long* __restrict__ prev_score, int prev_nq) {
    const int lane = threadIdx.x & 63, wave = threadIdx.x >> 6;
    for (int i = blockIdx.x * 256 + threadIdx.x; i < nlbox; i += gridDim.x * 256) lbox[i] = (i & 2) ? INT_MIN : INT_MAX;
    if (blockIdx.x == 0)
        for (int i = threadIdx.x; i < prev_nq; i += 256) {
            prev_score[i] = (long long)prev_sacc[16 * i];
            prev_sacc[16 * i] = 0ull;
        }
    const int r = lane >> 3, c4 = (lane & 7) * 4;
    const int sh = (r & 1) * 32 + c4;
    for (int item = blockIdx.x * 4 + wave; item < nq * g.nt; item += gridDim.x * 4) {
    const int q = item / g.nt, tile = item - q * g.nt;
    int c[4] = {0, 0, 0, 0};
    for (int s0 = 0; s0 < S; s0 += 16) {
        const int ls = s0 + (lane >> 2);
        const u64 mine = (ls < S) ? tcov[(((size_t)q * g.nt + tile) * S + ls) * 4 + (lane & 3)] : 0ull;
        if (__ballot(mine != 0ull) == 0) continue;

        const int ns = min(16, S - s0);
        for (int k = 0; k < ns; k++) {
            const int src = 4 * k + (r >> 1);
            const unsigned lo = (unsigned)__shfl((int)(unsigned)mine, src, 64), hi = (unsigned)__shfl((int)(unsigned)(mine >> 32), src, 64);
            const unsigned bits = (unsigned)(((((u64)hi) << 32) | lo) >> sh) & 15u;
#pragma unroll
            for (int j = 0; j < 4; j++) c[j] += (bits >> j) & 1u;
        }
    }
    int v = 0;
#pragma unroll
    for (int j = 0; j < 4; j++) v += c[j] * (S - c[j]);
#pragma unroll
    for (int o = 32; o > 0; o >>= 1) v += __shfl_xor(v, o, 64);
    if (lane == 0 && v) atomicAdd(&sacc[16 * q], (unsigned long long)v);
    if (count_img) {
        const int tx = tile % g.ntx, ty = tile / g.ntx;
        const int ix = tx * EHR_TILE_W + c4, iy = ty * EHR_TILE_H + r;
        if (iy < g.H)
#pragma unroll
            for (int j = 0; j < 4; j++)
                if (ix + j < g.W && c[j]) count_img[((size_t)q * g.H + (g.H - 1 - iy)) * g.W + ix + j] = (unsigned char)c[j];
    }
    }
}

static_assert(EHR_TILE_W == 32 && EHR_TILE_H == 8, "coverage words: four u64 per tile, word r >> 1 holds row r at bit (r & 1) * 32 + col");

__global__ void __launch_bounds__(256)
vb_overlap_pack_ref_kernel(BinGeom g, const float* __restrict__ ref, u64* __restrict__ rbits,
                           unsigned long long* __restrict__ ref_area) {
    const int lane = threadIdx.x & 63, wave = threadIdx.x >> 6, s = blockIdx.y;
    const int r = lane >> 3, c4 = (lane & 7) * 4;
    const int sh = (r & 1) * 32 + c4;
    const float* const img = ref + (size_t)s * g.H * g.W;
    unsigned n = 0;
    for (int tile = blockIdx.x * 4 + wave; tile < g.nt; tile += gridDim.x * 4) {
        const int tx = tile % g.ntx, ty = tile / g.ntx;
        const int ix = tx * EHR_TILE_W + c4, iy = ty * EHR_TILE_H + r;
        unsigned bits = 0;
        if (iy < g.H) {
            const float* const row = img + (size_t)(g.H - 1 - iy) * g.W;
#pragma unroll
            for (int j = 0; j < 4; j++)
                if (ix + j < g.W && row[ix + j] > 0.5f) bits |= 1u << j;
        }
        u64 w = (u64)bits << sh;
#pragma unroll
        for (int o = 1; o < 16; o <<= 1) w |= __shfl_xor(w, o, 64);
        if ((lane & 15) == 0) {
            rbits[((size_t)s * g.nt + tile) * 4 + (lane >> 4)] = w;
            n += __popcll(w);
        }
    }
#pragma unroll
    for (int o = 32; o > 0; o >>= 1) n += __shfl_xor(n, o, 64);
    if (lane == 0 && n) atomicAdd(&ref_area[s], (unsigned long long)n);
}

__global__ void __launch_bounds__(256)
vb_overlap_count_kernel(BinGeom g, int nq, int S, int per_wave, const u64* __restrict__ tcov, const u64* __restrict__ rbits,
                        unsigned long long* __restrict__ oacc, int* __restrict__ lbox, int nlbox,
                        unsigned long long* __restrict__ prev_oacc, long long* __restrict__ prev_out, int prev_n) {
    const int lane = threadIdx.x & 63, wave = threadIdx.x >> 6;
    for (int i = blockIdx.x * 256 + threadIdx.x; i < nlbox; i += gridDim.x * 256) lbox[i] = (i & 2) ? INT_MIN : INT_MAX;
    if (blockIdx.x == 0)
        for (int i = threadIdx.x; i < prev_n; i += 256) {
            const unsigned long long v = prev_oacc[16 * (size_t)i];
            prev_out[2 * (size_t)i] = (long long)(v & 0xffffffffull);
            prev_out[2 * (size_t)i + 1] = (long long)(v >> 32);
            prev_oacc[16 * (size_t)i] = 0ull;
        }
    const long long total = (long long)nq * g.nt;
    const long long first = (long long)(blockIdx.x * 4 + wave) * per_wave;
    if (first >= total) return;
    const int i0 = (int)first, i1 = (int)min(total, first + per_wave);
    const int k = lane & 3;
    for (int s0 = 0; s0 < S; s0 += 16) {
        const int ls = s0 + (lane >> 2);
        const bool on = ls < S;
        const u64* const cov = tcov + (size_t)(on ? ls : 0) * 4 + k;
        const u64* const rb = rbits + (size_t)(on ? ls : 0) * g.nt * 4 + k;
        unsigned inter = 0, area = 0;
        int q = i0 / g.nt, tile = i0 - q * g.nt;
        auto flush = [&]() {
            inter += __shfl_xor(inter, 1, 64);
            inter += __shfl_xor(inter, 2, 64);
            area += __shfl_xor(area, 1, 64);
            area += __shfl_xor(area, 2, 64);
            if (k == 0 && area) atomicAdd(&oacc[16 * ((size_t)q * S + ls)], ((unsigned long long)area << 32) | inter);
            inter = area = 0;
        };
        for (int i = i0; i < i1; i += 4) {
            u64 m[4];
#pragma unroll
            for (int j = 0; j < 4; j++) m[j] = (on && i + j < i1) ? cov[(size_t)(i + j) * S * 4] : 0ull;
#pragma unroll
            for (int j = 0; j < 4; j++) {
                if (i + j >= i1) break;
                if (__ballot(m[j] != 0ull) != 0) {
                    const u64 rw = on ? rb[(size_t)tile * 4] : 0ull;
                    area += __popcll(m[j]);
                    inter += __popcll(m[j] & rw);
                }
                if (++tile == g.nt) {
                    flush();
                    tile = 0;
                    q++;
                }
            }
        }
        if (tile != 0) flush();
    }
}

__global__ void vb_pad_kernel(const int32_t* __restrict__ a, int T, int4* __restrict__ out) {
    const int t = blockIdx.x * blockDim.x + threadIdx.x;
    if (t < T) out[t] = make_int4(a[3 * t], a[3 * t + 1], a[3 * t + 2], 0);
}

}
using namespace ehr;


static void vb_kd_order(const float* cen, int* idx, int n) {
    if (n <= 64) return;
    float lo[3] = {3.4e38f, 3.4e38f, 3.4e38f}, hi[3] = {-3.4e38f, -3.4e38f, -3.4e38f};
    for (int i = 0; i < n; i++)
        for (int k = 0; k < 3; k++) {
            const float c = cen[3 * (size_t)idx[i] + k];
            lo[k] = std::min(lo[k], c);
            hi[k] = std::max(hi[k], c);
        }
    int ax = 0;
    if (hi[1] - lo[1] > hi[ax] - lo[ax]) ax = 1;
    if (hi[2] - lo[2] > hi[ax] - lo[ax]) ax = 2;
    const int half = std::min(std::max(((n / 2 + 63) / 64) * 64, 64), n - 1);
    std::nth_element(idx, idx + half, idx + n, [&](int a, int b) {
        const float ca = cen[3 * (size_t)a + ax], cb = cen[3 * (size_t)b + ax];
        return ca < cb || (ca == cb && a < b);
    });
    vb_kd_order(cen, idx, half);
    vb_kd_order(cen, idx + half, n - half);
}

static int vb_build_clusters(Scratch& out, int& nc_out, int L, int V, int T, const float* verts, const int32_t* tris,
                             const int32_t* tri_link, const int32_t* vert_link = nullptr, bool* mixed = nullptr) {
    std::vector<float> hv((size_t)3 * std::max(V, 1));
    std::vector<int32_t> ht((size_t)3 * std::max(T, 1)), hl((size_t)std::max(T, 1));
    if (V > 0) EHR_HIP(hipMemcpy(hv.data(), verts, (size_t)3 * V * sizeof(float), hipMemcpyDeviceToHost));
    if (T > 0) {
        EHR_HIP(hipMemcpy(ht.data(), tris, (size_t)3 * T * sizeof(int32_t), hipMemcpyDeviceToHost));
        if (tri_link) {
            EHR_HIP(hipMemcpy(hl.data(), tri_link, (size_t)T * sizeof(int32_t), hipMemcpyDeviceToHost));
        } else {
            std::vector<int32_t> vl((size_t)std::max(V, 1), 0);
            if (V > 0) EHR_HIP(hipMemcpy(vl.data(), vert_link, (size_t)V * sizeof(int32_t), hipMemcpyDeviceToHost));
            int prev = 0;
            for (int t = 0; t < T; t++) {
                int lk[3];
                for (int j = 0; j < 3; j++) {
                    const int v = ht[3 * (size_t)t + j];
                    lk[j] = ((unsigned)v < (unsigned)V) ? vl[v] : -1;
                }
                if (lk[0] != lk[1] || lk[0] != lk[2] || (unsigned)lk[0] >= (unsigned)L || lk[0] < prev) {
                    *mixed = true;
                    return EHR_OK;
                }
                prev = lk[0];
                hl[t] = lk[0];
            }
        }
    }
    std::vector<int32_t> ctri, clink, coff((size_t)L + 1, 0);
    std::vector<float> aabb((size_t)6 * L);
    for (int l = 0; l < L; l++)
        for (int k = 0; k < 3; k++) {
            aabb[6 * (size_t)l + k] = 3.4e38f;
            aabb[6 * (size_t)l + 3 + k] = -3.4e38f;
        }
    int t = 0;
    for (int l = 0; l < L; l++) {
        coff[l] = (int32_t)clink.size();
        const int t0 = t;
        while (t < T && hl[t] == l) t++;
        if (t < T && hl[t] < l) return fail(EHR_ERR_INVALID, "ehr_fused_plan: tri_link must be sorted by link");
        const int n = t - t0;
        if (n == 0) continue;
        std::vector<float> cen((size_t)3 * n);
        float lo[3] = {3.4e38f, 3.4e38f, 3.4e38f}, hi[3] = {-3.4e38f, -3.4e38f, -3.4e38f};
        for (int i = 0; i < n; i++)
            for (int k = 0; k < 3; k++) {
                float c = 0.f;
                for (int j = 0; j < 3; j++) {
                    const int v = ht[3 * (size_t)(t0 + i) + j];
                    const float x = ((unsigned)v < (unsigned)V) ? hv[3 * (size_t)v + k] : 0.f;
                    c += x;
                    if ((unsigned)v < (unsigned)V) {
                        aabb[6 * (size_t)l + k] = std::min(aabb[6 * (size_t)l + k], x);
                        aabb[6 * (size_t)l + 3 + k] = std::max(aabb[6 * (size_t)l + 3 + k], x);
                    }
                }
                c *= (1.f / 3.f);
                if (!(c == c)) c = 0.f;
                cen[3 * (size_t)i + k] = c;
                lo[k] = std::min(lo[k], c);
                hi[k] = std::max(hi[k], c);
            }
        std::vector<int> order((size_t)n);
        for (int i = 0; i < n; i++) order[i] = i;
        vb_kd_order(cen.data(), order.data(), n);
        for (int i = 0; i < n; i++) {
            if ((i & 63) == 0) clink.push_back(l);
            ctri.push_back(t0 + order[i]);
        }
        while (ctri.size() & 63) ctri.push_back(-1);
    }
    if (t != T) return fail(EHR_ERR_INVALID, "ehr_fused_plan: tri_link holds a link outside [0, %d) or is not sorted", L);
    coff[L] = (int32_t)clink.size();
    const int NC = (int)clink.size();
    nc_out = NC;
    int rc;
    const size_t n_ctri = (size_t)std::max(NC, 1) * 64;
    std::vector<float> cvert(12 * n_ctri, 0.f);
    for (size_t i = 0; i < ctri.size(); i++) {
        const int tt = ctri[i];
        if (tt < 0) continue;
        const int v0 = ht[3 * (size_t)tt], v1 = ht[3 * (size_t)tt + 1], v2 = ht[3 * (size_t)tt + 2];
        if ((unsigned)v0 >= (unsigned)V || (unsigned)v1 >= (unsigned)V || (unsigned)v2 >= (unsigned)V) continue;
        const float c9[9] = {hv[3 * (size_t)v0], hv[3 * (size_t)v0 + 1], hv[3 * (size_t)v0 + 2], hv[3 * (size_t)v1], hv[3 * (size_t)v1 + 1],
                             hv[3 * (size_t)v1 + 2], hv[3 * (size_t)v2], hv[3 * (size_t)v2 + 1], hv[3 * (size_t)v2 + 2]};
        for (int k = 0; k < 4; k++) cvert[4 * i + k] = c9[k];
        for (int k = 0; k < 4; k++) cvert[4 * (n_ctri + i) + k] = c9[4 + k];
        cvert[4 * (2 * n_ctri + i)] = c9[8];
        cvert[4 * (2 * n_ctri + i) + 1] = 1.f;
    }
    std::vector<int32_t> cvidx(4 * n_ctri, 0);
    for (size_t i = 0; i < n_ctri; i++) {
        const int tt = i < ctri.size() ? ctri[i] : -1;
        cvidx[4 * i + 3] = tt;
        if (tt < 0) continue;
        for (int k = 0; k < 3; k++) {
            const int v = ht[3 * (size_t)tt + k];
            cvidx[4 * i + k] = ((unsigned)v < (unsigned)V) ? v : 0;
        }
    }
    for (int l = 0; l < L; l++)
        if (coff[l + 1] - coff[l] > 4096)
            return fail(EHR_ERR_INVALID, "ehr_fused_plan: link %d has more than 262144 triangles", l);
    if ((rc = out.reserve((n_ctri + std::max(NC, 1) + L + 1 + 6 * (size_t)L) * sizeof(int32_t) + 32 + cvert.size() * sizeof(float) +
                          cvidx.size() * sizeof(int32_t)))) return rc;
    int32_t* d = (int32_t*)out.ptr;
    if (NC > 0) {
        EHR_HIP(hipMemcpy(d, ctri.data(), (size_t)NC * 64 * sizeof(int32_t), hipMemcpyHostToDevice));
        EHR_HIP(hipMemcpy(d + n_ctri, clink.data(), (size_t)NC * sizeof(int32_t), hipMemcpyHostToDevice));
    }
    EHR_HIP(hipMemcpy(d + n_ctri + std::max(NC, 1), coff.data(), ((size_t)L + 1) * sizeof(int32_t), hipMemcpyHostToDevice));
    EHR_HIP(hipMemcpy(d + n_ctri + std::max(NC, 1) + L + 1, aabb.data(), aabb.size() * sizeof(float), hipMemcpyHostToDevice));
    {
        const uintptr_t at = ((uintptr_t)(d + n_ctri + std::max(NC, 1) + L + 1 + 6 * (size_t)L) + 15) & ~(uintptr_t)15;
        EHR_HIP(hipMemcpy((void*)at, cvert.data(), cvert.size() * sizeof(float), hipMemcpyHostToDevice));
        EHR_HIP(hipMemcpy((char*)at + cvert.size() * sizeof(float), cvidx.data(), cvidx.size() * sizeof(int32_t), hipMemcpyHostToDevice));
    }
    return EHR_OK;
}

static std::pair<VbClusters, VbSlotIdx> vb_cluster_index(const Scratch& scratch, int NC, int L) {
    const int NC1 = std::max(NC, 1);
    VbClusters cl;
    cl.ctri = (const int32_t*)scratch.ptr;
    cl.clink = cl.ctri + (size_t)NC1 * 64;
    cl.coff = cl.clink + NC1;
    cl.laabb = (const float*)(cl.coff + L + 1);
    cl.cvert = (const float4*)(((uintptr_t)(cl.laabb + 6 * (size_t)L) + 15) & ~(uintptr_t)15);
    cl.NC = NC;
    VbSlotIdx si;
    si.cvidx = (const int4*)(cl.cvert + 3 * (size_t)NC1 * 64);
    return {cl, si};
}

struct VbVertexGrid {
    int gx, xcd_views;
};
static VbVertexGrid vb_vertex_grid(int num_cus, int nitems, int Bk) {
    const int per_view_cap = std::max(8, (num_cus * VB_VERTEX_GRID) / std::max(Bk, 1));
    const int items_per_wg = (nitems + per_view_cap - 1) / per_view_cap;
    VbVertexGrid v;
    v.gx = std::max(1, (nitems + items_per_wg - 1) / std::max(items_per_wg, 1));
    v.xcd_views = (VB_XCD_SPLIT && (Bk % VB_XCDS) == 0) ? Bk / VB_XCDS : 0;
    return v;
}

int ehr::vbuf_plan(ehr_ctx* ctx, int B, int L, int V, int T, int H, int W, float slack, const float* verts,
                   const int32_t* tris, const int32_t* tri_link, const int32_t* opp) {
    if (H > 32760 || W > 32736)
        return fail(EHR_ERR_INVALID, "ehr_fused_plan: resolution above 32736 x 32760 (W x H) is unsupported");
    if ((V > 0 && !verts) || (T > 0 && (!tris || !tri_link || !opp)))
        return fail(EHR_ERR_INVALID, "ehr_fused_plan: the scene arrays (verts, tris, tri_link, opp) are required");
    int rc;
    if ((rc = vb_build_clusters(ctx->vb_clus, ctx->vb_nc, L, V, T, verts, tris, tri_link))) return rc;
    const int NC = std::max(ctx->vb_nc, 1);
    BinGeom gp = make_geom(H, W, L);
    const double jobs_per_view = std::max(1.0, ((slack > 0.f) ? std::min((double)L, (double)slack) : (double)L) * gp.nt);
    const double view_bytes = jobs_per_view * VB_SLOT_BYTES + (double)NC * VB_CLUSTER_REC_BYTES + (double)std::max(V, 1) * sizeof(float4) +
                              (double)L * gp.nt * sizeof(int);
    static const double budget = getenv("EHR_VB_SCRATCH_MB") ? atof(getenv("EHR_VB_SCRATCH_MB")) * 1048576.0 : 24576.0 * 1048576.0;
    int Bc = std::min(B, std::max(1, VB_MAX_UNITS / L));
    Bc = std::max(1, std::min(Bc, (int)(budget / view_bytes)));
    if (jobs_per_view * Bc > 2.0e9) return fail(EHR_ERR_INVALID, "ehr_fused_plan: views x links x tiles of a chunk exceeds 2e9");
    ctx->vb_chunk = Bc;
    if ((rc = ctx->vb_acc.reserve((size_t)B * vb_acc_stride(L) * sizeof(long long) + VB_META_BYTES))) return rc;
    {
        const char* e = getenv("EHR_VB_LAZY");
        ctx->vb_lazy = e ? atoi(e) != 0 : (double)V > 1.5 * (double)std::max(T, 1);
        if (ctx->vb_lazy != (ctx->vb_posc.ptr == nullptr) && ctx->gexec) {
            EHR_HIP(hipGraphExecDestroy(ctx->gexec));
            ctx->gexec = nullptr;
        }
        if (!ctx->vb_lazy && (rc = ctx->vb_posc.reserve((size_t)Bc * std::max(V, 1) * sizeof(float4)))) return rc;
    }
    size_t bytes;
    vb_recs(nullptr, Bc, NC, &bytes);
    if ((rc = ctx->vb_boxes.reserve(bytes))) return rc;
    {
        const char* e = getenv("EHR_VB_SPILL_ITEMS");
        ctx->vb_spill_cap = e ? std::max(0, atoi(e)) : VB_SPILL_ITEMS;
        if ((rc = ctx->vb_spill.reserve(std::max((size_t)ctx->vb_spill_cap * sizeof(VbItem), (size_t)1 << 20)))) return rc;
    }
    if ((rc = ctx->vb_units.reserve((size_t)VB_LBOX_STRIDE * B * L * sizeof(int)))) return rc;
    {
        if ((rc = ctx->vb_refsum.reserve(((size_t)B * gp.nt + B + 1) * sizeof(long long)))) return rc;
        ctx->vb_ref = nullptr;
        ctx->vb_weight = nullptr;
        ctx->vb_weight_views = 0;
    }
    ctx->vb_jcap = (int)(jobs_per_view * Bc);
    vb_slots(nullptr, (size_t)ctx->vb_jcap, (size_t)Bc * L, &bytes);
    if ((rc = ctx->vb_jobs.reserve(bytes))) return rc;
    vb_heavy(nullptr, (size_t)Bc * L * gp.nt, &bytes);
    if ((rc = ctx->vb_heavy.reserve(bytes))) return rc;
    EHR_HIP(hipMemset(ctx->vb_heavy.ptr, 0, bytes));
    if ((rc = ctx->vb_idx.reserve((size_t)2 * std::max(T, 1) * sizeof(int4)))) return rc;
    if (T > 0) {
        vb_pad_kernel<<<(T + 255) / 256, 256>>>(tris, T, (int4*)ctx->vb_idx.ptr);
        vb_pad_kernel<<<(T + 255) / 256, 256>>>(opp, T, (int4*)ctx->vb_idx.ptr + T);
        EHR_LAUNCH_CHECK();
    }
    if (!ctx->vb_hstate.ptr) {
        if ((rc = ctx->vb_hstate.reserve(16 * sizeof(int)))) return rc;
        EHR_HIP(hipMemset(ctx->vb_hstate.ptr, 0, 16 * sizeof(int)));
    }
    if (ctx->vb_hstate_m.cap < (size_t)VB_HSTATE_INTS * B * sizeof(int)) {
        if ((rc = ctx->vb_hstate_m.reserve((size_t)VB_HSTATE_INTS * B * sizeof(int)))) return rc;
        EHR_HIP(hipMemset(ctx->vb_hstate_m.ptr, 0, ctx->vb_hstate_m.cap));
    }
    ctx->vb_plan_tris = tris;
    ctx->vb_plan_opp = opp;
    ctx->vb_plan_verts = verts;
    EHR_HIP(hipMemset(ctx->vb_acc.ptr, 0, ctx->vb_acc.cap));
    std::vector<int> boxes((size_t)VB_LBOX_STRIDE * B * L);
    for (size_t i = 0; i < boxes.size(); i++) boxes[i] = (i & 2) ? INT_MIN : INT_MAX;
    EHR_HIP(hipMemcpy(ctx->vb_units.ptr, boxes.data(), boxes.size() * sizeof(int), hipMemcpyHostToDevice));
    EHR_HIP(hipDeviceSynchronize());
    return EHR_OK;
}

int ehr::vbuf_meta_read(ehr_ctx* ctx, int* meta4) {
    EHR_HIP(hipMemcpy(meta4, vb_acc_meta((long long*)ctx->vb_acc.ptr, ctx->pB, ctx->pL), 4 * sizeof(int), hipMemcpyDeviceToHost));
    return EHR_OK;
}

int ehr::vbuf_chain(ehr_ctx* ctx, const float* verts, const int32_t* tris, const int32_t* vert_link, const int32_t* opp, float* mvp, const float* ref, int B, int L, int V,
                    int T, int H, int W, float* mask, float* loss, float* grad_mvp, const StepHead* head,
                    const StepTail* tail, hipStream_t stream, int multi_views) {
    const bool multi = multi_views > 0;
    if (tris != ctx->vb_plan_tris || opp != ctx->vb_plan_opp || verts != ctx->vb_plan_verts)
        return fail(EHR_ERR_INVALID, "fused op: the scene arrays differ from the planned ones; call ehr_fused_plan again");
    BinGeom g = make_geom(H, W, L);
    long long* const facc_all = (long long*)ctx->vb_acc.ptr;
    const int acc_stride = vb_acc_stride(L);
    int* meta = vb_acc_meta(facc_all, B, L);
    int* const lbox_all = (int*)ctx->vb_units.ptr;
    VbItem* spill = (VbItem*)ctx->vb_spill.ptr;
    const int NC = ctx->vb_nc, NC1 = std::max(NC, 1);
    const auto [cl, si] = vb_cluster_index(ctx->vb_clus, NC, L);
    const int Bc = std::max(1, std::min(ctx->vb_chunk, B));
    VbHeavy hv = vb_heavy(ctx->vb_heavy.ptr, (size_t)Bc * L * g.nt);

    hipEvent_t* ev = nullptr;
    if (ctx->timing) {
        const size_t need = ctx->ev_used + EHR_FUSED_STAGES + 1;
        while (ctx->ev.size() < need) {
            hipEvent_t e;
            EHR_HIP(hipEventCreate(&e));
            ctx->ev.push_back(e);
        }
        ev = ctx->ev.data() + ctx->ev_used;
        ctx->ev_used = need;
        EHR_HIP(hipEventRecord(ev[0], stream));
    }
    const float* const weight = ctx->vb_weight;
    const int vec_ok = ((W & 3) == 0) && (((uintptr_t)ref & 15) == 0) && (!mask || ((uintptr_t)mask & 15) == 0) &&
                       (((uintptr_t)weight & 15) == 0);
    const int job_wgs = vb_xcd_round_up(ctx->num_cus * VB_JOB_GRID);
    hv.mcap = std::min(VB_MED_CAP, 2 * job_wgs);
    hv.heavy_base = VB_HEAVY_T_DEFAULT;
    hv.heavy_max = job_wgs / 2;
    const bool sparse = ctx->vb_ref != nullptr && ctx->vb_ref == ref && ctx->vb_ref_views == (multi ? multi_views : B);
    const long long* const tsum_all = sparse ? (const long long*)ctx->vb_refsum.ptr : nullptr;
    const long long* const vtot_all = sparse ? tsum_all + (size_t)B * g.nt : nullptr;
    const int* const ref_flag = sparse ? (const int*)(vtot_all + B) : nullptr;
    const bool with_slow = !tail || ctx->vb_slow_needed;
    VbSlots sl = vb_slots(ctx->vb_jobs.ptr, (size_t)ctx->vb_jcap, (size_t)Bc * L);
    if (!with_slow) sl.slow_list = nullptr;
    const bool lazy = ctx->vb_lazy;
    float4* const posc = lazy ? nullptr : (float4*)ctx->vb_posc.ptr;
    const int nvb = lazy ? 0 : (std::max(V, 1) + 255) / 256;
    const int nitems = nvb + (NC + 3) / 4;
    for (int b0 = 0; b0 < B; b0 += Bc) {
        const int Bk = std::min(Bc, B - b0);
        const bool first_chunk = b0 == 0, last_chunk = b0 + Bk == B;
        const bool time_it = ev && last_chunk;
        long long* facc = facc_all + (size_t)b0 * acc_stride;
        int* lbox = lbox_all + (size_t)VB_LBOX_STRIDE * b0 * L;
        float* mvp_k = mvp + (size_t)b0 * L * 16;
        const float* ref_k = multi ? ref : ref + (size_t)b0 * H * W;
        float* mask_k = mask ? mask + (size_t)b0 * H * W : nullptr;
        const VbRecs recs = vb_recs(ctx->vb_boxes.ptr, Bk, NC1);
        const VbVertexGrid vg = vb_vertex_grid(ctx->num_cus, nitems, Bk);
        const dim3 vgrid(vg.gx * Bk);
        const int nacc_ints = 2 * Bk * acc_stride;
        const int role = first_chunk ? VB_ROLE_FIRST_CHUNK : VB_ROLE_LATER_CHUNK;
        if (head && multi) {
            StepHead hk = *head;
            hk.view0 = b0;
            hk.nviews = multi_views;
            vb_vertex_kernel<true, true><<<vgrid, 256, 0, stream>>>(verts, vert_link, tris, cl, hk, mvp_k, V, nvb, g, posc, recs, lbox,
                                                                   (int*)facc, nacc_ints, meta, Bk, vg.gx, vg.xcd_views, hv, role);
        } else if (head) {
            StepHead hk = *head;
            hk.link_poses = head->link_poses + (size_t)b0 * L * 16;
            vb_vertex_kernel<true><<<vgrid, 256, 0, stream>>>(verts, vert_link, tris, cl, hk, mvp_k, V, nvb, g, posc, recs, lbox,
                                                             (int*)facc, nacc_ints, meta, Bk, vg.gx, vg.xcd_views, hv, role);
        } else {
            StepHead none = {};
            vb_vertex_kernel<false><<<vgrid, 256, 0, stream>>>(verts, vert_link, tris, cl, none, mvp_k, V, nvb, g, posc, recs,
                                                              lbox, (int*)facc, nacc_ints, meta, Bk, vg.gx, vg.xcd_views, hv, role);
        }
        EHR_LAUNCH_CHECK();
        if (time_it) EHR_HIP(hipEventRecord(ev[1], stream));
        VbResolveArgs rq;
        rq.verts = verts; rq.mvp = mvp_k; rq.posc = posc; rq.V = V; rq.L = L; rq.W = W; rq.H = H;
        rq.tri4 = (const int4*)ctx->vb_idx.ptr;
        rq.opp4 = (const int4*)ctx->vb_idx.ptr + T;
        rq.T = T;
        rq.sl = sl;
        rq.spill = spill;
        rq.spill_cap = ctx->vb_spill_cap;
        rq.meta = meta;
        rq.want_grad = grad_mvp ? 1 : 0;
        VbJobParams jp = {};
        jp.g = g; jp.B = Bk; jp.cl = cl; jp.si = si; jp.rc = recs; jp.lbox = lbox; jp.hv = hv;
        jp.use_hint = Bc == B;
        jp.heavy_t = VB_HEAVY_T_DEFAULT;
        jp.med_t0 = VB_MED_T_DEFAULT;
        jp.rq = rq;
        if (lazy)
            vb_job_kernel<false, true><<<job_wgs, 256, 0, stream>>>(jp);
        else
            vb_job_kernel<false><<<job_wgs, 256, 0, stream>>>(jp);
        EHR_LAUNCH_CHECK();
        if (with_slow) {
            vb_slow_kernel<<<VB_SLOW_GRID, 256, 0, stream>>>(rq, recs, cl.NC, si.cvidx, cl.coff);
            EHR_LAUNCH_CHECK();
        }
        if (time_it) {
            for (int k = 2; k <= 4; k++) EHR_HIP(hipEventRecord(ev[k], stream));
        }
        int nwg = ctx->num_cus * VB_COMPOSITE_GRID;
        if (!sparse) nwg = std::min(nwg, (Bk * g.nt + 3) / 4);
        nwg = std::max(VB_XCDS, vb_xcd_round_up(nwg));
        const size_t dyn = (2 * (size_t)Bk * L + 1) * sizeof(int);
        const bool fill = sparse && mask_k != nullptr;
        VbCompArgs ca;
        ca.g = g; ca.B = Bk; ca.mvp = mvp_k; ca.V = V; ca.verts = verts; ca.sl = sl; ca.ref = ref_k; ca.mask = mask_k; ca.facc = facc;
        ca.nls = VB_LOSS_SLOTS; ca.want_grad = rq.want_grad; ca.vec_ok = vec_ok; ca.spill = spill; ca.spill_cap = ctx->vb_spill_cap;
        ca.meta = meta;
        ca.tsum = sparse ? tsum_all + (size_t)b0 * g.nt : nullptr;
        ca.ref_flag = ref_flag; ca.loss = loss; ca.grad_mvp = grad_mvp;
        ca.do_finish = (last_chunk && !multi) ? 1 : 0; ca.B_all = B; ca.facc_all = facc_all; ca.vtot_all = vtot_all; ca.lbox_all = lbox_all;
        const VbWeight wt = {weight, b0, weight ? ctx->vb_weight_views : 1};
#define VB_COMPOSITE_W(TAILV, FILLV, SHAREDV, tailarg, sharg)                                                      \
    do {                                                                                                             \
        if (weight)                                                                                                  \
            vb_composite_kernel<TAILV, FILLV, SHAREDV, true><<<nwg, 256, dyn, stream>>>(ca, tailarg, sharg, wt);     \
        else                                                                                                         \
            vb_composite_kernel<TAILV, FILLV, SHAREDV><<<nwg, 256, dyn, stream>>>(ca, tailarg, sharg, wt);           \
    } while (0)
#define VB_COMPOSITE(TAILV, FILLV, tailarg) VB_COMPOSITE_W(TAILV, FILLV, false, tailarg, (VbSharedRef{0, 1}))
        StepTail none = {};
        if (multi) {
            const VbSharedRef sh = {b0, multi_views};
            if (fill)
                VB_COMPOSITE_W(false, true, true, none, sh);
            else
                VB_COMPOSITE_W(false, false, true, none, sh);
        } else if (tail) {
            if (fill) VB_COMPOSITE(true, true, *tail); else VB_COMPOSITE(true, false, *tail);
        } else {
            if (fill) VB_COMPOSITE(false, true, none); else VB_COMPOSITE(false, false, none);
        }
#undef VB_COMPOSITE
#undef VB_COMPOSITE_W
        EHR_LAUNCH_CHECK();
    }
    if (ev) EHR_HIP(hipEventRecord(ev[5], stream));
    if (multi) {
        MultiFinish mf;
        mf.facc_all = facc_all; mf.vtot_all = vtot_all; mf.ref_flag = ref_flag; mf.loss = loss; mf.grad_mvp = grad_mvp;
        mf.meta = meta; mf.lbox_all = lbox_all; mf.P = B / multi_views; mf.Bv = multi_views; mf.nls = VB_LOSS_SLOTS; mf.g = g;
        vb_finish_multi_kernel<<<mf.P, 256, 0, stream>>>(mf, *tail);
        EHR_LAUNCH_CHECK();
    }
    if (ev) {
        for (int k = 6; k <= 7; k++) EHR_HIP(hipEventRecord(ev[k], stream));
    }
    return EHR_OK;
}

struct VbScoreMisc {
    int* lbox;
    int* meta;
    VbHeavy hv;
    int* sticky;
    size_t zero_bytes;
    unsigned long long* sacc;
    u64* tcov;
    void* own;
};
static VbScoreMisc vb_score_misc(void* base, size_t Qc, size_t Bc, int L, int nt, size_t own_bytes, size_t* bytes = nullptr) {
    VbCarve c{(uintptr_t)base};
    VbScoreMisc m;
    m.lbox = c.take<int>((size_t)VB_LBOX_STRIDE * Bc * L);
    m.meta = (int*)c.take<char>(VB_META_BYTES, alignof(int));
    size_t hv_bytes;
    m.hv = vb_heavy((void*)c.at, 0, &hv_bytes);
    c.at += hv_bytes;
    m.hv.stamp = m.hv.gen;
    m.sticky = c.take<int>(16);
    m.zero_bytes = c.at - (uintptr_t)m.hv.gen;
    m.sacc = c.take<unsigned long long>(2 * 16 * Qc, 128);
    m.tcov = c.take<u64>(Bc * nt * 4);
    m.own = c.take<char>(own_bytes, 128);
    if (bytes) *bytes = c.at - (uintptr_t)base;
    return m;
}

struct VbOverlapMisc {
    unsigned long long* oacc;
    u64* rbits;
};
static VbOverlapMisc vb_overlap_misc(void* base, size_t Bc, int S, int nt, size_t* bytes = nullptr) {
    VbCarve c{(uintptr_t)base};
    VbOverlapMisc m;
    m.oacc = c.take<unsigned long long>(2 * 16 * Bc, 128);
    m.rbits = c.take<u64>((size_t)S * nt * 4, 128);
    if (bytes) *bytes = c.at - (uintptr_t)base;
    return m;
}

struct VbCovChunk {
    BinGeom g;
    int S, Qc, Bc, nlbox, num_cus;
    VbScoreMisc m;
};

template <class Stage>
static int vb_cov_chain(ehr_ctx* ctx, const float* verts, const int32_t* tris, const int32_t* vert_link, const float* mvp, int Q,
                        int S, int L, int V, int T, int H, int W, hipStream_t stream, int* handled, Stage& st) {
    *handled = 0;
    const char* const want = getenv("EHR_SCORE_PATH");
    const bool must = want && !strcmp(want, "chain");
    if (want && !strcmp(want, "tile")) return EHR_OK;
    if (!vert_link || L > 32 || S * L > VB_MAX_UNITS || H > 32760 || W > 32736)
        return must ? fail(EHR_ERR_INVALID, "%s: EHR_SCORE_PATH=chain, but the call's sizes do not allow it", st.op) : EHR_OK;
    int rc;
    unsigned long long hash = 0;
    {
        if ((rc = ctx->sc_misc.reserve(4096))) return rc;
        unsigned long long* dh = (unsigned long long*)ctx->sc_misc.ptr;
        EHR_HIP(hipMemsetAsync(dh, 0, sizeof(unsigned long long), stream));
        vb_hash_kernel<<<64, 256, 0, stream>>>((const unsigned*)verts, (size_t)3 * V, (const unsigned*)tris, (size_t)3 * T,
                                                (const unsigned*)vert_link, (size_t)V, dh);
        EHR_LAUNCH_CHECK();
        EHR_HIP(hipMemcpyAsync(ctx->host_pinned, dh, sizeof(unsigned long long), hipMemcpyDeviceToHost, stream));
        EHR_HIP(hipStreamSynchronize(stream));
        hash = *(unsigned long long*)ctx->host_pinned;
    }
    if (ctx->sc_key[0] != verts || ctx->sc_key[1] != tris || ctx->sc_key[2] != vert_link || ctx->sc_key_n[0] != V ||
        ctx->sc_key_n[1] != T || ctx->sc_key_n[2] != L || ctx->sc_hash != hash) {
        bool mixed = false;
        ctx->sc_key[0] = nullptr;
        if ((rc = vb_build_clusters(ctx->sc_clus, ctx->sc_nc, L, V, T, verts, tris, nullptr, vert_link, &mixed))) {
            if (rc == EHR_ERR_INVALID) return EHR_OK;
            return rc;
        }
        ctx->sc_mixed = mixed;
        ctx->sc_key[0] = verts;
        ctx->sc_key[1] = tris;
        ctx->sc_key[2] = vert_link;
        ctx->sc_key_n[0] = V;
        ctx->sc_key_n[1] = T;
        ctx->sc_key_n[2] = L;
        ctx->sc_hash = hash;
    }
    if (ctx->sc_mixed || ctx->sc_nc <= 0)
        return must ? fail(EHR_ERR_INVALID, "%s: EHR_SCORE_PATH=chain, but the mesh's links are not grouped", st.op) : EHR_OK;
    VbCovChunk c;
    c.g = make_geom(H, W, L);
    const BinGeom& g = c.g;
    const int NC = ctx->sc_nc;
    const auto [cl, si] = vb_cluster_index(ctx->sc_clus, NC, L);
    const double view_bytes = (double)NC * VB_CLUSTER_REC_BYTES + (double)V * sizeof(float4) + (double)g.nt * 4 * sizeof(u64);
    int Qc = std::max(1, (VB_MAX_UNITS / L) / S);
    Qc = std::max(1, std::min(Qc, (int)(8192.0 * 1048576.0 / (view_bytes * S))));
    Qc = std::min(Qc, Q);
    const int Bc = Qc * S;
    size_t bytes;
    if ((rc = ctx->sc_posc.reserve((size_t)Bc * V * sizeof(float4)))) return rc;
    vb_recs(nullptr, Bc, NC, &bytes);
    if ((rc = ctx->sc_entries.reserve(bytes))) return rc;
    const size_t own_bytes = st.own_bytes(Bc, g.nt);
    vb_score_misc(nullptr, Qc, Bc, L, g.nt, own_bytes, &bytes);
    if ((rc = ctx->sc_misc.reserve(bytes))) return rc;
    ctx->sc_entries_cap = 0;
    c.m = vb_score_misc(ctx->sc_misc.ptr, Qc, Bc, L, g.nt, own_bytes);
    c.S = S; c.Qc = Qc; c.Bc = Bc; c.nlbox = VB_LBOX_STRIDE * Bc * L; c.num_cus = ctx->num_cus;
    const VbScoreMisc& m = c.m;
    float4* posc = (float4*)ctx->sc_posc.ptr;
    EHR_HIP(hipMemsetAsync(m.hv.gen, 0, m.zero_bytes, stream));
    const int nvb = (std::max(V, 1) + 255) / 256;
    const int nitems = nvb + (NC + 3) / 4;
    const int job_wgs = vb_xcd_round_up(ctx->num_cus * VB_JOB_GRID);
    if ((rc = st.begin(c, stream))) return rc;
    for (int q0 = 0; q0 < Q; q0 += Qc) {
        const int nq = std::min(Qc, Q - q0), Bk = nq * S;
        const VbRecs recs = vb_recs(ctx->sc_entries.ptr, Bk, NC);
        const VbVertexGrid vg = vb_vertex_grid(ctx->num_cus, nitems, Bk);
        StepHead none = {};
        vb_vertex_kernel<false><<<dim3(vg.gx * Bk), 256, 0, stream>>>(verts, vert_link, tris, cl, none, const_cast<float*>(mvp) + (size_t)q0 * S * L * 16,
                                                                   V, nvb, g, posc, recs, m.lbox, (int*)m.tcov, Bk * g.nt * 8, m.meta, Bk, vg.gx,
                                                                   vg.xcd_views, m.hv, VB_ROLE_FIRST_CHUNK | VB_ROLE_POS_ONLY);
        EHR_LAUNCH_CHECK();
        VbJobParams jp = {};
        jp.g = g; jp.B = Bk; jp.cl = cl; jp.si = si; jp.rc = recs; jp.lbox = m.lbox; jp.hv = m.hv;
        jp.rq.verts = verts; jp.rq.posc = posc; jp.rq.V = V; jp.rq.meta = m.meta;
        jp.rq.mvp = mvp + (size_t)q0 * S * L * 16;
        jp.co = {m.tcov, m.sticky, S};
        jp.heavy_t = 0x7fffffff;
        jp.med_t0 = 0x7fffffff;
        vb_job_kernel<true><<<job_wgs, 256, 0, stream>>>(jp);
        EHR_LAUNCH_CHECK();
        if ((rc = st.chunk(c, q0, nq, stream))) return rc;
    }
    if ((rc = st.end(c, stream))) return rc;
    EHR_HIP(hipMemcpyAsync(ctx->host_pinned, m.sticky, sizeof(int), hipMemcpyDeviceToHost, stream));
    EHR_HIP(hipMemcpyAsync(ctx->host_pinned + 1, m.meta + EHR_META_OVERFLOW, sizeof(int), hipMemcpyDeviceToHost, stream));
    EHR_HIP(hipStreamSynchronize(stream));
    if (ctx->host_pinned[0] || ctx->host_pinned[1])
        return must ? fail(EHR_ERR_INVALID, "%s: EHR_SCORE_PATH=chain, but a triangle needs the exact z-buffer", st.op) : EHR_OK;
    *handled = 1;
    return EHR_OK;
}

struct VbVarianceStage {
    const char* op = "ehr_mask_variance";
    long long* score;
    unsigned char* count;
    int Q, H, W;
    unsigned long long* prev_sacc = nullptr;
    long long* prev_score = nullptr;
    int prev_nq = 0, flip = 0;
    size_t own_bytes(int, int) const { return 0; }
    int begin(const VbCovChunk& c, hipStream_t stream) {
        EHR_HIP(hipMemsetAsync(c.m.sacc, 0, 2 * 16 * (size_t)c.Qc * sizeof(unsigned long long), stream));
        EHR_HIP(hipMemsetAsync(score, 0, (size_t)Q * sizeof(long long), stream));
        if (count) EHR_HIP(hipMemsetAsync(count, 0, (size_t)Q * H * W, stream));
        vb_score_count_kernel<<<64, 256, 0, stream>>>(c.g, 0, c.S, c.m.tcov, c.m.sacc, nullptr, c.m.lbox, c.nlbox, c.m.sacc, score, 0);
        EHR_LAUNCH_CHECK();
        prev_sacc = c.m.sacc;
        prev_score = score;
        return EHR_OK;
    }
    int chunk(const VbCovChunk& c, int q0, int nq, hipStream_t stream) {
        unsigned long long* const sacc = c.m.sacc + (size_t)flip * 16 * c.Qc;
        vb_score_count_kernel<<<std::min((nq * c.g.nt + 3) / 4, VB_SCORE_COUNT_GRID * c.num_cus), 256, 0, stream>>>(
            c.g, nq, c.S, c.m.tcov, sacc, count ? count + (size_t)q0 * H * W : nullptr, c.m.lbox, c.nlbox, prev_sacc, prev_score, prev_nq);
        EHR_LAUNCH_CHECK();
        prev_sacc = sacc;
        prev_score = score + q0;
        prev_nq = nq;
        flip ^= 1;
        return EHR_OK;
    }
    int end(const VbCovChunk& c, hipStream_t stream) {
        vb_score_count_kernel<<<1, 256, 0, stream>>>(c.g, 0, c.S, c.m.tcov, c.m.sacc, nullptr, c.m.lbox, 0, prev_sacc, prev_score, prev_nq);
        EHR_LAUNCH_CHECK();
        return EHR_OK;
    }
};

int ehr::vbuf_score(ehr_ctx* ctx, const float* verts, const int32_t* tris, const int32_t* vert_link, const float* mvp, int Q,
                    int S, int L, int V, int T, int H, int W, long long* score, unsigned char* count, hipStream_t stream,
                    int* handled) {
    VbVarianceStage st;
    st.score = score; st.count = count; st.Q = Q; st.H = H; st.W = W;
    return vb_cov_chain(ctx, verts, tris, vert_link, mvp, Q, S, L, V, T, H, W, stream, handled, st);
}

constexpr int VB_OVERLAP_WAVE_ITEMS = 32;
struct VbOverlapStage {
    const char* op = "ehr_mask_overlap";
    const float* ref;
    long long* overlap;
    long long* ref_area;
    int Q, S;
    VbOverlapMisc o = {};
    unsigned long long* prev_oacc = nullptr;
    long long* prev_out = nullptr;
    int prev_n = 0, flip = 0;
    size_t own_bytes(int Bc, int nt) const {
        size_t bytes;
        vb_overlap_misc(nullptr, Bc, S, nt, &bytes);
        return bytes;
    }
    int begin(const VbCovChunk& c, hipStream_t stream) {
        o = vb_overlap_misc(c.m.own, c.Bc, c.S, c.g.nt);
        EHR_HIP(hipMemsetAsync(o.oacc, 0, 2 * 16 * (size_t)c.Bc * sizeof(unsigned long long), stream));
        EHR_HIP(hipMemsetAsync(overlap, 0, (size_t)Q * c.S * 2 * sizeof(long long), stream));
        EHR_HIP(hipMemsetAsync(ref_area, 0, (size_t)c.S * sizeof(long long), stream));
        vb_overlap_pack_ref_kernel<<<dim3(std::min((c.g.nt + 3) / 4, 16), c.S), 256, 0, stream>>>(c.g, ref, o.rbits,
                                                                                                  (unsigned long long*)ref_area);
        EHR_LAUNCH_CHECK();
        vb_overlap_count_kernel<<<64, 256, 0, stream>>>(c.g, 0, c.S, 1, c.m.tcov, o.rbits, o.oacc, c.m.lbox, c.nlbox, o.oacc, overlap, 0);
        EHR_LAUNCH_CHECK();
        prev_oacc = o.oacc;
        prev_out = overlap;
        return EHR_OK;
    }
    int chunk(const VbCovChunk& c, int q0, int nq, hipStream_t stream) {
        unsigned long long* const oacc = o.oacc + (size_t)flip * 16 * c.Bc;
        const long long total = (long long)nq * c.g.nt;
        const long long max_waves = 4ll * VB_SCORE_COUNT_GRID * c.num_cus;
        const int per_wave = (int)std::max<long long>(VB_OVERLAP_WAVE_ITEMS, (total + max_waves - 1) / max_waves);
        const int wgs = (int)((total + 4ll * per_wave - 1) / (4ll * per_wave));
        vb_overlap_count_kernel<<<wgs, 256, 0, stream>>>(c.g, nq, c.S, per_wave, c.m.tcov, o.rbits, oacc, c.m.lbox, c.nlbox, prev_oacc,
                                                         prev_out, prev_n);
        EHR_LAUNCH_CHECK();
        prev_oacc = oacc;
        prev_out = overlap + (size_t)q0 * c.S * 2;
        prev_n = nq * c.S;
        flip ^= 1;
        return EHR_OK;
    }
    int end(const VbCovChunk& c, hipStream_t stream) {
        vb_overlap_count_kernel<<<1, 256, 0, stream>>>(c.g, 0, c.S, 1, c.m.tcov, o.rbits, o.oacc, c.m.lbox, 0, prev_oacc, prev_out, prev_n);
        EHR_LAUNCH_CHECK();
        return EHR_OK;
    }
};

int ehr::vbuf_overlap(ehr_ctx* ctx, const float* verts, const int32_t* tris, const int32_t* vert_link, const float* mvp,
                      const float* ref, int Q, int S, int L, int V, int T, int H, int W, long long* overlap, long long* ref_area,
                      hipStream_t stream, int* handled) {
    VbOverlapStage st;
    st.ref = ref; st.overlap = overlap; st.ref_area = ref_area; st.Q = Q; st.S = S;
    return vb_cov_chain(ctx, verts, tris, vert_link, mvp, Q, S, L, V, T, H, W, stream, handled, st);
}

int ehr::vbuf_bind_ref(ehr_ctx* ctx, const float* ref, int views, hipStream_t stream) {
    ctx->vb_ref = nullptr;
    if (!ref) return EHR_OK;
    const int B = ctx->pB, H = ctx->pH, W = ctx->pW;
    if (views <= 0 || B % views != 0) return fail(EHR_ERR_INVALID, "ehr_fused_bind_ref: the plan's %d views are not a multiple of %d", B, views);
    BinGeom g = make_geom(H, W, ctx->pL);
    long long* tsum = (long long*)ctx->vb_refsum.ptr;
    long long* vtot = tsum + (size_t)B * g.nt;
    EHR_HIP(hipMemsetAsync(vtot, 0, ((size_t)B + 1) * sizeof(long long), stream));
    const float* const weight = ctx->vb_weight;
    const int vec_ok = ((W & 3) == 0) && (((uintptr_t)ref & 15) == 0) && (((uintptr_t)weight & 15) == 0);
    const int nw = views * g.nt;
    for (int b0 = 0; b0 < B; b0 += views) {
        const VbWeight wt = {weight, b0, weight ? ctx->vb_weight_views : 1};
        if (weight)
            vb_refsum_kernel<true><<<(nw + 3) / 4, 256, 0, stream>>>(g, views, ref, vec_ok, tsum + (size_t)b0 * g.nt, vtot + b0, (int*)(vtot + B), wt);
        else
            vb_refsum_kernel<false><<<(nw + 3) / 4, 256, 0, stream>>>(g, views, ref, vec_ok, tsum + (size_t)b0 * g.nt, vtot + b0, (int*)(vtot + B), wt);
        EHR_LAUNCH_CHECK();
    }
    ctx->vb_ref = ref;
    ctx->vb_ref_views = views;
    return EHR_OK;
}
```

### include/ehr.h

```cpp
#ifndef EHR_H
#define EHR_H

#include <stddef.h>
#include <stdint.h>

#ifdef __cplusplus
extern "C" {
#endif

#define EHR_OK 0
#define EHR_ERR_INVALID (-1)
#define EHR_ERR_HIP (-2)
#define EHR_ERR_OVERFLOW (-3)
#define EHR_ERR_RETRY (-4)

typedef struct ehr_ctx ehr_ctx;

int ehr_version(void);
const char* ehr_last_error(void);
int ehr_device_count(void);
const char* ehr_device_arch(int dev);

int ehr_ctx_create(int device, ehr_ctx** out);
int ehr_ctx_destroy(ehr_ctx* ctx);
size_t ehr_ctx_scratch_bytes(ehr_ctx* ctx);

size_t ehr_tile_flags_bytes(int B, int H, int W);
int ehr_rasterize_fwd(ehr_ctx* ctx, const float* pos, const int32_t* tri, const int32_t* ranges_host, int B, int V,
                      int T, int H, int W, float* rast, float* rast_db, unsigned char* tile_flags, void* stream);

int ehr_rasterize_grad(const float* pos, const int32_t* tri, const float* rast, const float* dy, int range_mode, int B,
                       int V, int T, int H, int W, float* grad_pos, const unsigned char* tile_flags, void* stream);
int ehr_rasterize_grad_db(const float* pos, const int32_t* tri, const float* rast, const float* ddb, int range_mode, int B,
                          int V, int T, int H, int W, float* grad_pos, void* stream);

int ehr_interpolate_fwd(const float* attr, const float* rast, const int32_t* tri, int B, int Ba, int V, int T, int A,
                        int H, int W, float* out, const unsigned char* tile_flags, void* stream);
int ehr_interpolate_grad(const float* attr, const float* rast, const int32_t* tri, const float* dy, int B, int Ba, int V,
                         int T, int A, int H, int W, float* grad_attr, float* grad_rast, const unsigned char* tile_flags,
                         void* stream);

int ehr_interpolate_da_fwd(const float* attr, const float* rast, const float* rast_db, const int32_t* tri,
                           const int32_t* diff_idx, int B, int Ba, int V, int T, int A, int D, int H, int W, float* out_da,
                           void* stream);
int ehr_interpolate_da_grad(const float* attr, const float* rast, const float* rast_db, const int32_t* tri,
                            const int32_t* diff_idx, const float* dy_da, int B, int Ba, int V, int T, int A, int D, int H,
                            int W, float* grad_attr, float* grad_rast_db, void* stream);

size_t ehr_topology_scratch_bytes(int T);
int ehr_antialias_topology(const int32_t* tri, int T, int32_t* opp, void* scratch, size_t scratch_bytes, void* stream);

size_t ehr_antialias_work_bytes(int B, int H, int W);
int ehr_antialias_fwd(const float* color, const float* rast, const float* pos, const int32_t* tri, const int32_t* opp,
                      int range_mode, int B, int V, int T, int H, int W, int C, float* out, void* work,
                      const unsigned char* tile_flags, void* stream);
int ehr_antialias_fwd_zg(const float* color, const float* rast, const float* pos, const int32_t* tri, const int32_t* opp,
                         int range_mode, int B, int V, int T, int H, int W, int C, float* out, void* work,
                         const unsigned char* tile_flags, float* grad_pos_zero, void* stream);
int ehr_antialias_grad(const float* color, const float* rast, const float* pos, const int32_t* tri, const float* dy,
                       const void* work, int range_mode, int B, int V, int T, int H, int W, int C, float* grad_color,
                       float* grad_pos, void* stream);

int ehr_fused_plan(ehr_ctx* ctx, int B, int L, int V, int T, int H, int W, float slack, const float* verts,
                   const int32_t* tris, const int32_t* tri_link, const int32_t* opp);
int ehr_render_mask_loss(ehr_ctx* ctx, const float* verts, const int32_t* tris, const int32_t* tri_link,
                         const int32_t* vert_link, const int32_t* opp, const float* mvp, const float* ref, int B,
                         int L, int V, int T, int H, int W, float* mask, float* loss, float* grad_mvp, void* stream);
int ehr_fused_status(ehr_ctx* ctx);

int ehr_fused_bind_ref(ehr_ctx* ctx, const float* ref, void* stream);
int ehr_fused_bind_ref_shared(ehr_ctx* ctx, const float* ref, int Bv, void* stream);

int ehr_fused_bind_weight(ehr_ctx* ctx, const float* weight, int Bv, void* stream);

#define EHR_FUSED_STAGES 7
int ehr_fused_timing(ehr_ctx* ctx, int enable);
int ehr_fused_timing_read(ehr_ctx* ctx, float* ms, int* ncalls);

int ehr_pose_forward(const float* dof, const float* K, const float* link_poses, int B, int L, int H, int W, float n,
                     float f, float* mvp, float* tc_jac, const int32_t* step, float* history, int history_rows,
                     void* stream);
int ehr_pose_backward(const float* grad_mvp, const float* loss, const float* K, const float* link_poses,
                      const float* tc_jac, int B, int L, int H, int W, float n, float f, float* red, void* stream);
int ehr_pose_adam(float* dof, float* m, float* v, int32_t* step, const float* red, float lr, float beta1, float beta2,
                  float eps, float weight_decay, float* loss_out, float* grad_out, void* stream);

int ehr_solver_step(ehr_ctx* ctx, const float* verts, const int32_t* tris, const int32_t* tri_link,
                    const int32_t* vert_link, const int32_t* opp, const float* K, const float* link_poses,
                    const float* ref, int B, int L, int V, int T, int H, int W, float near_plane, float far_plane,
                    float* dof, float* adam_m, float* adam_v, int32_t* step, float* history, int history_rows,
                    int32_t* history_row, float lr, float beta1, float beta2, float eps, float weight_decay, float* mvp,
                    float* tc_jac, float* mask, float* loss_b, float* grad_mvp, float* red, float* loss_out,
                    float* grad_out, int defer_adam, void* stream);

int ehr_solver_step_multi(ehr_ctx* ctx, const float* verts, const int32_t* tris, const int32_t* tri_link,
                          const int32_t* vert_link, const int32_t* opp, const float* K, const float* link_poses,
                          const float* ref, int P, int Bv, int L, int V, int T, int H, int W, float near_plane,
                          float far_plane, float* dof, float* adam_m, float* adam_v, int32_t* step, float* history,
                          int history_rows, int32_t* history_row, float lr, float beta1, float beta2, float eps,
                          float weight_decay, float* mvp, float* tc_jac, float* mask, float* loss_b, float* grad_mvp,
                          float* red, float* loss_out, float* grad_out, void* stream);

int ehr_comm_unique_id(void* id128_host);
int ehr_comm_init(ehr_ctx* ctx, const void* id128_host, int nranks, int rank);
int ehr_comm_allreduce(ehr_ctx* ctx, float* red, int count, void* stream);
int ehr_comm_destroy(ehr_ctx* ctx);

#define EHR_P2P_MAX_RANKS 64
int ehr_comm_p2p_export(ehr_ctx* ctx, void* handle64_host);
int ehr_comm_p2p_open(ehr_ctx* ctx, const void* handles_host, int nranks, int rank);
int ehr_comm_p2p_step(ehr_ctx* ctx, float* red, float* dof, float* m, float* v, int32_t* step, float lr, float beta1,
                      float beta2, float eps, float weight_decay, float* loss_out, float* grad_out, void* stream);
int ehr_comm_p2p_close(ehr_ctx* ctx);

int ehr_graph_begin(ehr_ctx* ctx, void** capture_stream);
int ehr_graph_end(ehr_ctx* ctx);
int ehr_graph_launch(ehr_ctx* ctx, void* stream);
int ehr_graph_release(ehr_ctx* ctx);

int ehr_mask_variance(ehr_ctx* ctx, const float* verts, const int32_t* tris, const int32_t* vert_link,
                      const float* mvp, int Q, int S, int L, int V, int T, int H, int W, int64_t* score,
                      uint8_t* count, int chunk_views, void* stream);

int ehr_mask_overlap(ehr_ctx* ctx, const float* verts, const int32_t* tris, const int32_t* vert_link, const float* mvp,
                     const float* ref, int Q, int S, int L, int V, int T, int H, int W, int64_t* overlap,
                     int64_t* ref_area, int chunk_views, void* stream);

int ehr_joint_forward(const int32_t* parent, const double* origin, const int32_t* kind, const double* axis,
                      const int32_t* qidx, const int32_t* use, int N, int J, int L, const double* qpos, const float* offset,
                      int B, float* link_poses, float* joint_frames, void* stream);
int ehr_joint_backward_adam(const float* grad_mvp, const float* tc_jac, const float* K, int B, int L, int J, int H, int W,
                            float near_plane, float far_plane, const float* link_poses, const float* joint_frames,
                            const uint32_t* upstream, const int32_t* joint_kind, const float* red, const int32_t* free_joints,
                            float* offset, float* adam_m, float* adam_v, int32_t* step_j, float lr, float beta1, float beta2,
                            float eps, float weight_decay, float* grad_out, void* stream);

#ifdef __cplusplus
}
#endif
#endif
```

Before: 116,500 frames/s.

## Share transformed vertices per cluster instead of per-triangle vertex copies

Replaces the per-triangle packed vertex copies (three positions per triangle slot) with a per-cluster unique vertex list plus per-triangle 8-bit indices. Each wave transforms and snaps each unique cluster vertex once into LDS and also writes the position cache for vertices it owns, so a separate pass only covers loose vertices. This removes redundant vertex transforms, snapping and cluster geometry bandwidth in the binning kernel. In exchange it adds LDS usage (float4 and int2 per vertex for four waves), a wave sync, a loop for clusters with more than 64 vertices, and a cap of 192 vertices per cluster.

```diff
diff --git a/easyhec_amd/_lib.py b/easyhec_amd/_lib.py
--- a/easyhec_amd/_lib.py
+++ b/easyhec_amd/_lib.py
@@ -40,6 +40,8 @@
                                    c_int, c_int, c_int, c_int, c_void_p, c_void_p, c_void_p]),
     "ehr_fused_plan": (c_int, [c_void_p, c_int, c_int, c_int, c_int, c_int, c_int, c_float, c_void_p, c_void_p,
                                 c_void_p, c_void_p]),
+    "ehr_fused_cluster_tables": (c_int, [c_int, c_int, c_int, c_void_p, c_void_p, c_void_p, ctypes.POINTER(c_int),
+                                          ctypes.POINTER(c_int), c_void_p, c_void_p, c_void_p, c_void_p, c_void_p]),
     "ehr_render_mask_loss": (c_int, [c_void_p, c_void_p, c_void_p, c_void_p, c_void_p, c_void_p, c_void_p, c_void_p,
                                      c_int, c_int, c_int, c_int, c_int, c_int, c_void_p, c_void_p, c_void_p,
                                      c_void_p]),
diff --git a/easyhec_amd/csrc/ehr_device.h b/easyhec_amd/csrc/ehr_device.h
--- a/easyhec_amd/csrc/ehr_device.h
+++ b/easyhec_amd/csrc/ehr_device.h
@@ -100,15 +100,19 @@
     bool valid;
 };
 
-__device__ __forceinline__ Coverage setup_coverage(const float4& a, const float4& b, const float4& c, int W, int H) {
+__device__ __forceinline__ int2 snap_vertex(const float4& a, int W, int H) {
+    const float sx = (float)(W * 8), sy = (float)(H * 8);
+    return make_int2(snap_coord(a.x, a.w, sx), snap_coord(a.y, a.w, sy));
+}
+
+__device__ __forceinline__ Coverage setup_coverage_snapped(const int2& a, const int2& b, const int2& c, int W, int H) {
     Coverage cv;
-    const float sx = (float)(W * 8), sy = (float)(H * 8);
-    cv.X[0] = snap_coord(a.x, a.w, sx);
-    cv.Y[0] = snap_coord(a.y, a.w, sy);
-    cv.X[1] = snap_coord(b.x, b.w, sx);
-    cv.Y[1] = snap_coord(b.y, b.w, sy);
-    cv.X[2] = snap_coord(c.x, c.w, sx);
-    cv.Y[2] = snap_coord(c.y, c.w, sy);
+    cv.X[0] = a.x;
+    cv.Y[0] = a.y;
+    cv.X[1] = b.x;
+    cv.Y[1] = b.y;
+    cv.X[2] = c.x;
+    cv.Y[2] = c.y;
     i64 area2 = (i64)(cv.X[1] - (i64)cv.X[0]) * (i64)(cv.Y[2] - (i64)cv.Y[0]) -
                 (i64)(cv.X[2] - (i64)cv.X[0]) * (i64)(cv.Y[1] - (i64)cv.Y[0]);
     cv.valid = area2 != 0;
@@ -134,6 +138,10 @@
     cv.iy1 = iy1;
     if (ix0 > ix1 || iy0 > iy1) cv.valid = false;
     return cv;
+}
+
+__device__ __forceinline__ Coverage setup_coverage(const float4& a, const float4& b, const float4& c, int W, int H) {
+    return setup_coverage_snapped(snap_vertex(a, W, H), snap_vertex(b, W, H), snap_vertex(c, W, H), W, H);
 }
 
 struct EdgeEval {
diff --git a/easyhec_amd/csrc/ehr_fused.hip b/easyhec_amd/csrc/ehr_fused.hip
--- a/easyhec_amd/csrc/ehr_fused.hip
+++ b/easyhec_amd/csrc/ehr_fused.hip
@@ -36,6 +36,13 @@
     ctx->pH = H;
     ctx->pW = W;
     return EHR_OK;
+}
+
+int ehr_fused_cluster_tables(int L, int V, int T, const float* verts, const int32_t* tris, const int32_t* tri_link, int* nc,
+                             int* nloose, int32_t* ctri, int32_t* cnv, uint32_t* cvl, uint32_t* ctl, int32_t* loose) {
+    if (L <= 0 || L > MAX_LINKS || V < 0 || T < 0 || !nc || !nloose || (V > 0 && !verts) || (T > 0 && (!tris || !tri_link)))
+        return fail(EHR_ERR_INVALID, "ehr_fused_cluster_tables: bad sizes (1 <= L <= %d) or a NULL array", MAX_LINKS);
+    return vbuf_cluster_tables(L, V, T, verts, tris, tri_link, nc, nloose, ctri, cnv, cvl, ctl, loose);
 }
 
 static int fused_chain(ehr_ctx* ctx, const float* verts, const int32_t* tris, const int32_t* tri_link,
diff --git a/easyhec_amd/csrc/ehr_host.h b/easyhec_amd/csrc/ehr_host.h
--- a/easyhec_amd/csrc/ehr_host.h
+++ b/easyhec_amd/csrc/ehr_host.h
@@ -56,6 +56,8 @@
 int vbuf_plan(ehr_ctx* ctx, int B, int L, int V, int T, int H, int W, float slack, const float* verts,
               const int32_t* tris, const int32_t* tri_link, const int32_t* opp);
 int vbuf_meta_read(ehr_ctx* ctx, int* meta4);
+int vbuf_cluster_tables(int L, int V, int T, const float* verts, const int32_t* tris, const int32_t* tri_link, int* nc, int* nuv,
+                        int32_t* ctri, int32_t* cnv, uint32_t* cvl, uint32_t* ctl, int32_t* uvl);
 int vbuf_bind_ref(ehr_ctx* ctx, const float* ref, int views, hipStream_t stream);
 int vbuf_score(ehr_ctx* ctx, const float* verts, const int32_t* tris, const int32_t* vert_link, const float* mvp, int Q, int S,
                int L, int V, int T, int H, int W, long long* score, unsigned char* count, hipStream_t stream, int* handled);
@@ -96,6 +98,7 @@
     const void* vb_plan_opp = nullptr;
     const void* vb_plan_verts = nullptr;
     int vb_nc = 0;
+    int vb_nuv = 0;
     int vb_jcap = 0;
     int vb_chunk = 0;
     ehr::Scratch vb_boxes;
@@ -118,6 +121,7 @@
     size_t sc_entries_cap = 0;
     ehr::Scratch sc_clus, sc_misc;
     int sc_nc = 0;
+    int sc_nuv = 0;
     const void* sc_key[3] = {nullptr, nullptr, nullptr};
     int sc_key_n[3] = {0, 0, 0};
     unsigned long long sc_hash = 0;
diff --git a/easyhec_amd/csrc/ehr_vbuf.hip b/easyhec_amd/csrc/ehr_vbuf.hip
--- a/easyhec_amd/csrc/ehr_vbuf.hip
+++ b/easyhec_amd/csrc/ehr_vbuf.hip
@@ -158,12 +158,18 @@
     return (int)((unsigned)id >> 22) * nt + ((id >> 10) & 4095) * ntx + (id & 1023);
 }
 static_assert(VB_MAX_UNITS <= 1024, "vb_hint_pack");
+constexpr int VB_CLUSTER_VERTS = 192;
+constexpr unsigned VB_CVL_OWNER = 0x80000000u;
+constexpr unsigned VB_CTL_DRAWS = 1u << 24;
 struct VbClusters {
     const int32_t* ctri;
     const int32_t* clink;
     const int32_t* coff;
     const float* laabb;
-    const float4* cvert;
+    const unsigned* cvl;
+    const unsigned* ctl;
+    const int32_t* uvl;
+    int nuv;
     int NC;
 };
 
@@ -287,39 +293,49 @@
     const bool first_head = MULTI ? (bx == 0 && bview == 0) : first;
     const int nitems = nvb + (cl.NC + 3) / 4;
     const int lane = tid & 63;
+    const int wave = tid >> 6;
     int item = bx;
-    int l = -1, t = -1;
-    float vx[3] = {0.f, 0.f, 0.f}, vy[3] = {0.f, 0.f, 0.f}, vz[3] = {0.f, 0.f, 0.f};
-    bool have = false;
+    int cw = -1, t = -1;
+    unsigned ve = ~0u;
+    int vl0 = -1;
+    unsigned tl = 0;
+    float vx = 0.f, vy = 0.f, vz = 0.f;
     auto load_geometry = [&](int it) {
-        l = -1;
+        cw = -1;
         t = -1;
-        have = false;
+        ve = ~0u;
+        vl0 = -1;
+        tl = 0;
         if (it < nvb) {
-            const int v = it * 256 + tid;
-            if (v < V) {
-                l = vert_link[v];
-                vx[0] = verts[3 * v];
-                vy[0] = verts[3 * v + 1];
-                vz[0] = verts[3 * v + 2];
-                have = true;
+            const int i = it * 256 + tid;
+            if (i < cl.nuv) {
+                ve = (unsigned)cl.uvl[i];
+                vl0 = vert_link[ve];
             }
         } else {
-            const int c = (it - nvb) * 4 + (tid >> 6);
+            const int c = (it - nvb) * 4 + wave;
             if (c < cl.NC) {
-                const size_t cs = (size_t)c * 64 + lane, cn = (size_t)cl.NC * 64;
+                const size_t cs = (size_t)c * 64 + lane;
                 t = cl.ctri[cs];
-                l = cl.clink[c];
-                const float4 q0 = cl.cvert[cs], q1 = cl.cvert[cn + cs], q2 = cl.cvert[2 * cn + cs];
-                vx[0] = q0.x; vy[0] = q0.y; vz[0] = q0.z;
-                vx[1] = q0.w; vy[1] = q1.x; vz[1] = q1.y;
-                vx[2] = q1.z; vy[2] = q1.w; vz[2] = q2.x;
-                have = t >= 0 && q2.y != 0.f;
-            }
+                cw = cl.clink[c];
+                tl = cl.ctl[cs];
+                if (lane < (cw >> 8)) {
+                    ve = cl.cvl[(size_t)c * VB_CLUSTER_VERTS + lane];
+                    if (posc && (ve & VB_CVL_OWNER)) vl0 = vert_link[ve & ~VB_CVL_OWNER];
+                }
+            }
+        }
+        if (ve != ~0u) {
+            const size_t v = ve & ~VB_CVL_OWNER;
+            vx = verts[3 * v];
+            vy = verts[3 * v + 1];
+            vz = verts[3 * v + 2];
         }
     };
     if (item < nitems) load_geometry(item);
     __shared__ int lacc[32][4];
+    __shared__ float4 vpos[4][VB_CLUSTER_VERTS];
+    __shared__ int2 vsnap[4][VB_CLUSTER_VERTS];
     if (tid < 128) lacc[tid >> 2][tid & 3] = (tid & 2) ? -1 : INT_MAX;
     __shared__ float LP[32][16];
     __shared__ float Kc[9];
@@ -427,23 +443,46 @@
     }
     __syncthreads();
     for (; item < nitems;) {
+    const int l = cw & 255, nv = min(cw >> 8, VB_CLUSTER_VERTS);
     const bool lv = (unsigned)l < (unsigned)L;
     if (item < nvb) {
-        const int v = item * 256 + tid;
-        if (v < V) {
+        if (ve != ~0u) {
             float4 o = make_float4(0.f, 0.f, 0.f, -1.f);
-            if (lv) o = transform_vertex(M[l], vx[0], vy[0], vz[0]);
-            posc[(size_t)b * V + v] = o;
+            if ((unsigned)vl0 < (unsigned)L) o = transform_vertex(M[vl0], vx, vy, vz);
+            posc[(size_t)b * V + ve] = o;
         }
     } else {
-    const int c = (item - nvb) * 4 + (tid >> 6);
+    const int c = (item - nvb) * 4 + wave;
     const bool cvalid = c < cl.NC;
     int x0 = 0xffff, y0 = 0xffff, x1 = 0, y1 = 0;
     int4 r0 = make_int4(-1, -1, -1, 0), r1 = make_int4(0, 0, t, 0);
-    if (have && lv) {
-        const float4 p0 = transform_vertex(M[l], vx[0], vy[0], vz[0]);
-        const float4 p1 = transform_vertex(M[l], vx[1], vy[1], vz[1]);
-        const float4 p2 = transform_vertex(M[l], vx[2], vy[2], vz[2]);
+    float4* const wpos = vpos[wave];
+    int2* const wsnap = vsnap[wave];
+    if (lv) {
+        for (int k = lane; k < nv; k += 64) {
+            if (k >= 64) ve = cl.cvl[(size_t)c * VB_CLUSTER_VERTS + k];
+            const bool own = posc && (ve & VB_CVL_OWNER);
+            const size_t v = ve & ~VB_CVL_OWNER;
+            if (k >= 64) {
+                vx = verts[3 * v];
+                vy = verts[3 * v + 1];
+                vz = verts[3 * v + 2];
+                if (own) vl0 = vert_link[v];
+            }
+            const float4 o = transform_vertex(M[l], vx, vy, vz);
+            wpos[k] = o;
+            wsnap[k] = snap_vertex(o, W, H);
+            if (own) {
+                float4 oo = o;
+                if (vl0 != l) oo = ((unsigned)vl0 < (unsigned)L) ? transform_vertex(M[vl0], vx, vy, vz) : make_float4(0.f, 0.f, 0.f, -1.f);
+                posc[(size_t)b * V + v] = oo;
+            }
+        }
+    }
+    VB_WAVE_SYNC();
+    if ((tl & VB_CTL_DRAWS) && lv) {
+        const int i0 = (int)(tl & 255u), i1 = (int)((tl >> 8) & 255u), i2 = (int)((tl >> 16) & 255u);
+        const float4 p0 = wpos[i0], p1 = wpos[i1], p2 = wpos[i2];
         const bool simple = (p0.w > 0.f) && (p1.w > 0.f) && (p2.w > 0.f) && (p0.z + p0.w >= 0.f) &&
                             (p1.z + p1.w >= 0.f) && (p2.z + p2.w >= 0.f);
         if (!simple) {
@@ -461,7 +500,7 @@
             }
             r1.w = 1;
         } else {
-            const Coverage cv = setup_coverage(p0, p1, p2, W, H);
+            const Coverage cv = setup_coverage_snapped(wsnap[i0], wsnap[i1], wsnap[i2], W, H);
             if (cv.valid) {
                 x0 = cv.ix0; y0 = cv.iy0; x1 = cv.ix1; y1 = cv.iy1;
                 const unsigned ex = (unsigned)max(cv.X[0], max(cv.X[1], cv.X[2])) - (unsigned)min(cv.X[0], min(cv.X[1], cv.X[2]));
@@ -2485,36 +2524,19 @@
     vb_kd_order(cen, idx + half, n - half);
 }
 
-static int vb_build_clusters(Scratch& out, int& nc_out, int L, int V, int T, const float* verts, const int32_t* tris,
-                             const int32_t* tri_link, const int32_t* vert_link = nullptr, bool* mixed = nullptr) {
-    std::vector<float> hv((size_t)3 * std::max(V, 1));
-    std::vector<int32_t> ht((size_t)3 * std::max(T, 1)), hl((size_t)std::max(T, 1));
-    if (V > 0) EHR_HIP(hipMemcpy(hv.data(), verts, (size_t)3 * V * sizeof(float), hipMemcpyDeviceToHost));
-    if (T > 0) {
-        EHR_HIP(hipMemcpy(ht.data(), tris, (size_t)3 * T * sizeof(int32_t), hipMemcpyDeviceToHost));
-        if (tri_link) {
-            EHR_HIP(hipMemcpy(hl.data(), tri_link, (size_t)T * sizeof(int32_t), hipMemcpyDeviceToHost));
-        } else {
-            std::vector<int32_t> vl((size_t)std::max(V, 1), 0);
-            if (V > 0) EHR_HIP(hipMemcpy(vl.data(), vert_link, (size_t)V * sizeof(int32_t), hipMemcpyDeviceToHost));
-            int prev = 0;
-            for (int t = 0; t < T; t++) {
-                int lk[3];
-                for (int j = 0; j < 3; j++) {
-                    const int v = ht[3 * (size_t)t + j];
-                    lk[j] = ((unsigned)v < (unsigned)V) ? vl[v] : -1;
-                }
-                if (lk[0] != lk[1] || lk[0] != lk[2] || (unsigned)lk[0] >= (unsigned)L || lk[0] < prev) {
-                    *mixed = true;
-                    return EHR_OK;
-                }
-                prev = lk[0];
-                hl[t] = lk[0];
-            }
-        }
-    }
-    std::vector<int32_t> ctri, clink, coff((size_t)L + 1, 0);
-    std::vector<float> aabb((size_t)6 * L);
+struct VbClusterTables {
+    std::vector<int32_t> ctri, clink, coff, cnv, uvl, cvidx;
+    std::vector<uint32_t> cvl, ctl;
+    std::vector<float> aabb;
+    int NC = 0;
+};
+static int vb_cluster_tables(VbClusterTables& tb, int L, int V, int T, const float* hv, const int32_t* ht, const int32_t* hl) {
+    std::vector<int32_t>&ctri = tb.ctri, &clink = tb.clink, &coff = tb.coff;
+    std::vector<float>& aabb = tb.aabb;
+    ctri.clear();
+    clink.clear();
+    coff.assign((size_t)L + 1, 0);
+    aabb.resize((size_t)6 * L);
     for (int l = 0; l < L; l++)
         for (int k = 0; k < 3; k++) {
             aabb[6 * (size_t)l + k] = 3.4e38f;
@@ -2560,64 +2582,138 @@
     if (t != T) return fail(EHR_ERR_INVALID, "ehr_fused_plan: tri_link holds a link outside [0, %d) or is not sorted", L);
     coff[L] = (int32_t)clink.size();
     const int NC = (int)clink.size();
-    nc_out = NC;
-    int rc;
+    tb.NC = NC;
     const size_t n_ctri = (size_t)std::max(NC, 1) * 64;
-    std::vector<float> cvert(12 * n_ctri, 0.f);
-    for (size_t i = 0; i < ctri.size(); i++) {
-        const int tt = ctri[i];
-        if (tt < 0) continue;
-        const int v0 = ht[3 * (size_t)tt], v1 = ht[3 * (size_t)tt + 1], v2 = ht[3 * (size_t)tt + 2];
-        if ((unsigned)v0 >= (unsigned)V || (unsigned)v1 >= (unsigned)V || (unsigned)v2 >= (unsigned)V) continue;
-        const float c9[9] = {hv[3 * (size_t)v0], hv[3 * (size_t)v0 + 1], hv[3 * (size_t)v0 + 2], hv[3 * (size_t)v1], hv[3 * (size_t)v1 + 1],
-                             hv[3 * (size_t)v1 + 2], hv[3 * (size_t)v2], hv[3 * (size_t)v2 + 1], hv[3 * (size_t)v2 + 2]};
-        for (int k = 0; k < 4; k++) cvert[4 * i + k] = c9[k];
-        for (int k = 0; k < 4; k++) cvert[4 * (n_ctri + i) + k] = c9[4 + k];
-        cvert[4 * (2 * n_ctri + i)] = c9[8];
-        cvert[4 * (2 * n_ctri + i) + 1] = 1.f;
-    }
-    std::vector<int32_t> cvidx(4 * n_ctri, 0);
+    tb.cnv.assign((size_t)std::max(NC, 1), 0);
+    tb.cvl.assign((size_t)std::max(NC, 1) * VB_CLUSTER_VERTS, 0u);
+    tb.ctl.assign(n_ctri, 0u);
+    {
+        std::vector<int32_t> seen((size_t)std::max(V, 1), -1), pos((size_t)std::max(V, 1), 0);
+        std::vector<char> owned((size_t)std::max(V, 1), 0);
+        for (size_t i = 0; i < ctri.size(); i++) {
+            const int tt = ctri[i], c = (int)(i >> 6);
+            if (tt < 0) continue;
+            const int vv[3] = {ht[3 * (size_t)tt], ht[3 * (size_t)tt + 1], ht[3 * (size_t)tt + 2]};
+            if ((unsigned)vv[0] >= (unsigned)V || (unsigned)vv[1] >= (unsigned)V || (unsigned)vv[2] >= (unsigned)V) continue;
+            uint32_t word = VB_CTL_DRAWS;
+            for (int k = 0; k < 3; k++) {
+                const int v = vv[k];
+                if (seen[v] != c) {
+                    seen[v] = c;
+                    pos[v] = tb.cnv[c]++;
+                    tb.cvl[(size_t)c * VB_CLUSTER_VERTS + pos[v]] = (uint32_t)v | (owned[v] ? 0u : VB_CVL_OWNER);
+                    owned[v] = 1;
+                }
+                word |= (uint32_t)pos[v] << (8 * k);
+            }
+            tb.ctl[i] = word;
+        }
+        tb.uvl.clear();
+        for (int v = 0; v < V; v++)
+            if (!owned[v]) tb.uvl.push_back(v);
+    }
+    tb.cvidx.assign(4 * n_ctri, 0);
     for (size_t i = 0; i < n_ctri; i++) {
         const int tt = i < ctri.size() ? ctri[i] : -1;
-        cvidx[4 * i + 3] = tt;
+        tb.cvidx[4 * i + 3] = tt;
         if (tt < 0) continue;
         for (int k = 0; k < 3; k++) {
             const int v = ht[3 * (size_t)tt + k];
-            cvidx[4 * i + k] = ((unsigned)v < (unsigned)V) ? v : 0;
+            tb.cvidx[4 * i + k] = ((unsigned)v < (unsigned)V) ? v : 0;
         }
     }
     for (int l = 0; l < L; l++)
         if (coff[l + 1] - coff[l] > 4096)
             return fail(EHR_ERR_INVALID, "ehr_fused_plan: link %d has more than 262144 triangles", l);
-    if ((rc = out.reserve((n_ctri + std::max(NC, 1) + L + 1 + 6 * (size_t)L) * sizeof(int32_t) + 32 + cvert.size() * sizeof(float) +
-                          cvidx.size() * sizeof(int32_t)))) return rc;
-    int32_t* d = (int32_t*)out.ptr;
-    if (NC > 0) {
-        EHR_HIP(hipMemcpy(d, ctri.data(), (size_t)NC * 64 * sizeof(int32_t), hipMemcpyHostToDevice));
-        EHR_HIP(hipMemcpy(d + n_ctri, clink.data(), (size_t)NC * sizeof(int32_t), hipMemcpyHostToDevice));
-    }
-    EHR_HIP(hipMemcpy(d + n_ctri + std::max(NC, 1), coff.data(), ((size_t)L + 1) * sizeof(int32_t), hipMemcpyHostToDevice));
-    EHR_HIP(hipMemcpy(d + n_ctri + std::max(NC, 1) + L + 1, aabb.data(), aabb.size() * sizeof(float), hipMemcpyHostToDevice));
-    {
-        const uintptr_t at = ((uintptr_t)(d + n_ctri + std::max(NC, 1) + L + 1 + 6 * (size_t)L) + 15) & ~(uintptr_t)15;
-        EHR_HIP(hipMemcpy((void*)at, cvert.data(), cvert.size() * sizeof(float), hipMemcpyHostToDevice));
-        EHR_HIP(hipMemcpy((char*)at + cvert.size() * sizeof(float), cvidx.data(), cvidx.size() * sizeof(int32_t), hipMemcpyHostToDevice));
-    }
     return EHR_OK;
 }
 
-static std::pair<VbClusters, VbSlotIdx> vb_cluster_index(const Scratch& scratch, int NC, int L) {
-    const int NC1 = std::max(NC, 1);
+static std::pair<VbClusters, VbSlotIdx> vb_cluster_carve(void* base, int NC, int L, int nuv, size_t* bytes = nullptr) {
+    const size_t NC1 = (size_t)std::max(NC, 1);
+    VbCarve c{(uintptr_t)base};
     VbClusters cl;
-    cl.ctri = (const int32_t*)scratch.ptr;
-    cl.clink = cl.ctri + (size_t)NC1 * 64;
-    cl.coff = cl.clink + NC1;
-    cl.laabb = (const float*)(cl.coff + L + 1);
-    cl.cvert = (const float4*)(((uintptr_t)(cl.laabb + 6 * (size_t)L) + 15) & ~(uintptr_t)15);
+    cl.ctri = c.take<int32_t>(NC1 * 64);
+    cl.clink = c.take<int32_t>(NC1);
+    cl.coff = c.take<int32_t>((size_t)L + 1);
+    cl.laabb = c.take<float>(6 * (size_t)L);
+    cl.ctl = c.take<unsigned>(NC1 * 64);
+    cl.cvl = c.take<unsigned>(NC1 * VB_CLUSTER_VERTS);
+    cl.uvl = c.take<int32_t>((size_t)std::max(nuv, 1));
+    cl.nuv = nuv;
     cl.NC = NC;
     VbSlotIdx si;
-    si.cvidx = (const int4*)(cl.cvert + 3 * (size_t)NC1 * 64);
+    si.cvidx = c.take<int4>(NC1 * 64, 16);
+    if (bytes) *bytes = c.at - (uintptr_t)base;
     return {cl, si};
+}
+
+static int vb_build_clusters(Scratch& out, int& nc_out, int& nuv_out, int L, int V, int T, const float* verts, const int32_t* tris,
+                             const int32_t* tri_link, const int32_t* vert_link = nullptr, bool* mixed = nullptr) {
+    std::vector<float> hv((size_t)3 * std::max(V, 1));
+    std::vector<int32_t> ht((size_t)3 * std::max(T, 1)), hl((size_t)std::max(T, 1));
+    if (V > 0) EHR_HIP(hipMemcpy(hv.data(), verts, (size_t)3 * V * sizeof(float), hipMemcpyDeviceToHost));
+    if (T > 0) {
+        EHR_HIP(hipMemcpy(ht.data(), tris, (size_t)3 * T * sizeof(int32_t), hipMemcpyDeviceToHost));
+        if (tri_link) {
+            EHR_HIP(hipMemcpy(hl.data(), tri_link, (size_t)T * sizeof(int32_t), hipMemcpyDeviceToHost));
+        } else {
+            std::vector<int32_t> vl((size_t)std::max(V, 1), 0);
+            if (V > 0) EHR_HIP(hipMemcpy(vl.data(), vert_link, (size_t)V * sizeof(int32_t), hipMemcpyDeviceToHost));
+            int prev = 0;
+            for (int t = 0; t < T; t++) {
+                int lk[3];
+                for (int j = 0; j < 3; j++) {
+                    const int v = ht[3 * (size_t)t + j];
+                    lk[j] = ((unsigned)v < (unsigned)V) ? vl[v] : -1;
+                }
+                if (lk[0] != lk[1] || lk[0] != lk[2] || (unsigned)lk[0] >= (unsigned)L || lk[0] < prev) {
+                    *mixed = true;
+                    return EHR_OK;
+                }
+                prev = lk[0];
+                hl[t] = lk[0];
+            }
+        }
+    }
+    VbClusterTables tb;
+    int rc;
+    if ((rc = vb_cluster_tables(tb, L, V, T, hv.data(), ht.data(), hl.data()))) return rc;
+    const int NC = tb.NC, nuv = (int)tb.uvl.size();
+    nc_out = NC;
+    nuv_out = nuv;
+    size_t bytes;
+    vb_cluster_carve(nullptr, NC, L, nuv, &bytes);
+    if ((rc = out.reserve(bytes))) return rc;
+    const auto [cl, si] = vb_cluster_carve(out.ptr, NC, L, nuv);
+    if (NC > 0) {
+        EHR_HIP(hipMemcpy((void*)cl.ctri, tb.ctri.data(), (size_t)NC * 64 * sizeof(int32_t), hipMemcpyHostToDevice));
+        std::vector<int32_t> cw((size_t)NC);
+        for (int c = 0; c < NC; c++) cw[c] = tb.clink[c] | (tb.cnv[c] << 8);
+        EHR_HIP(hipMemcpy((void*)cl.clink, cw.data(), (size_t)NC * sizeof(int32_t), hipMemcpyHostToDevice));
+    }
+    EHR_HIP(hipMemcpy((void*)cl.coff, tb.coff.data(), ((size_t)L + 1) * sizeof(int32_t), hipMemcpyHostToDevice));
+    EHR_HIP(hipMemcpy((void*)cl.laabb, tb.aabb.data(), tb.aabb.size() * sizeof(float), hipMemcpyHostToDevice));
+    EHR_HIP(hipMemcpy((void*)cl.ctl, tb.ctl.data(), tb.ctl.size() * sizeof(uint32_t), hipMemcpyHostToDevice));
+    EHR_HIP(hipMemcpy((void*)cl.cvl, tb.cvl.data(), tb.cvl.size() * sizeof(uint32_t), hipMemcpyHostToDevice));
+    if (nuv > 0) EHR_HIP(hipMemcpy((void*)cl.uvl, tb.uvl.data(), (size_t)nuv * sizeof(int32_t), hipMemcpyHostToDevice));
+    EHR_HIP(hipMemcpy((void*)si.cvidx, tb.cvidx.data(), tb.cvidx.size() * sizeof(int32_t), hipMemcpyHostToDevice));
+    return EHR_OK;
+}
+
+int ehr::vbuf_cluster_tables(int L, int V, int T, const float* verts, const int32_t* tris, const int32_t* tri_link, int* nc,
+                             int* nuv, int32_t* ctri, int32_t* cnv, uint32_t* cvl, uint32_t* ctl, int32_t* uvl) {
+    VbClusterTables tb;
+    int rc;
+    if ((rc = vb_cluster_tables(tb, L, V, T, verts, tris, tri_link))) return rc;
+    *nc = tb.NC;
+    *nuv = (int)tb.uvl.size();
+    const size_t NC = (size_t)tb.NC;
+    if (ctri) std::copy(tb.ctri.begin(), tb.ctri.begin() + NC * 64, ctri);
+    if (cnv) std::copy(tb.cnv.begin(), tb.cnv.begin() + NC, cnv);
+    if (cvl) std::copy(tb.cvl.begin(), tb.cvl.begin() + NC * VB_CLUSTER_VERTS, cvl);
+    if (ctl) std::copy(tb.ctl.begin(), tb.ctl.begin() + NC * 64, ctl);
+    if (uvl) std::copy(tb.uvl.begin(), tb.uvl.end(), uvl);
+    return EHR_OK;
 }
 
 struct VbVertexGrid {
@@ -2639,7 +2735,7 @@
     if ((V > 0 && !verts) || (T > 0 && (!tris || !tri_link || !opp)))
         return fail(EHR_ERR_INVALID, "ehr_fused_plan: the scene arrays (verts, tris, tri_link, opp) are required");
     int rc;
-    if ((rc = vb_build_clusters(ctx->vb_clus, ctx->vb_nc, L, V, T, verts, tris, tri_link))) return rc;
+    if ((rc = vb_build_clusters(ctx->vb_clus, ctx->vb_nc, ctx->vb_nuv, L, V, T, verts, tris, tri_link))) return rc;
     const int NC = std::max(ctx->vb_nc, 1);
     BinGeom gp = make_geom(H, W, L);
     const double jobs_per_view = std::max(1.0, ((slack > 0.f) ? std::min((double)L, (double)slack) : (double)L) * gp.nt);
@@ -2724,7 +2820,7 @@
     int* const lbox_all = (int*)ctx->vb_units.ptr;
     VbItem* spill = (VbItem*)ctx->vb_spill.ptr;
     const int NC = ctx->vb_nc, NC1 = std::max(NC, 1);
-    const auto [cl, si] = vb_cluster_index(ctx->vb_clus, NC, L);
+    const auto [cl, si] = vb_cluster_carve(ctx->vb_clus.ptr, NC, L, ctx->vb_nuv);
     const int Bc = std::max(1, std::min(ctx->vb_chunk, B));
     VbHeavy hv = vb_heavy(ctx->vb_heavy.ptr, (size_t)Bc * L * g.nt);
 
@@ -2756,7 +2852,7 @@
     if (!with_slow) sl.slow_list = nullptr;
     const bool lazy = ctx->vb_lazy;
     float4* const posc = lazy ? nullptr : (float4*)ctx->vb_posc.ptr;
-    const int nvb = lazy ? 0 : (std::max(V, 1) + 255) / 256;
+    const int nvb = lazy ? 0 : (cl.nuv + 255) / 256;
     const int nitems = nvb + (NC + 3) / 4;
     for (int b0 = 0; b0 < B; b0 += Bc) {
         const int Bk = std::min(Bc, B - b0);
@@ -2942,7 +3038,7 @@
         ctx->sc_key_n[1] != T || ctx->sc_key_n[2] != L || ctx->sc_hash != hash) {
         bool mixed = false;
         ctx->sc_key[0] = nullptr;
-        if ((rc = vb_build_clusters(ctx->sc_clus, ctx->sc_nc, L, V, T, verts, tris, nullptr, vert_link, &mixed))) {
+        if ((rc = vb_build_clusters(ctx->sc_clus, ctx->sc_nc, ctx->sc_nuv, L, V, T, verts, tris, nullptr, vert_link, &mixed))) {
             if (rc == EHR_ERR_INVALID) return EHR_OK;
             return rc;
         }
@@ -2961,7 +3057,7 @@
     c.g = make_geom(H, W, L);
     const BinGeom& g = c.g;
     const int NC = ctx->sc_nc;
-    const auto [cl, si] = vb_cluster_index(ctx->sc_clus, NC, L);
+    const auto [cl, si] = vb_cluster_carve(ctx->sc_clus.ptr, NC, L, ctx->sc_nuv);
     const double view_bytes = (double)NC * VB_CLUSTER_REC_BYTES + (double)V * sizeof(float4) + (double)g.nt * 4 * sizeof(u64);
     int Qc = std::max(1, (VB_MAX_UNITS / L) / S);
     Qc = std::max(1, std::min(Qc, (int)(8192.0 * 1048576.0 / (view_bytes * S))));
@@ -2980,7 +3076,7 @@
     const VbScoreMisc& m = c.m;
     float4* posc = (float4*)ctx->sc_posc.ptr;
     EHR_HIP(hipMemsetAsync(m.hv.gen, 0, m.zero_bytes, stream));
-    const int nvb = (std::max(V, 1) + 255) / 256;
+    const int nvb = (cl.nuv + 255) / 256;
     const int nitems = nvb + (NC + 3) / 4;
     const int job_wgs = vb_xcd_round_up(ctx->num_cus * VB_JOB_GRID);
     if ((rc = st.begin(c, stream))) return rc;
diff --git a/include/ehr.h b/include/ehr.h
--- a/include/ehr.h
+++ b/include/ehr.h
@@ -63,6 +63,8 @@
 
 int ehr_fused_plan(ehr_ctx* ctx, int B, int L, int V, int T, int H, int W, float slack, const float* verts,
                    const int32_t* tris, const int32_t* tri_link, const int32_t* opp);
+int ehr_fused_cluster_tables(int L, int V, int T, const float* verts, const int32_t* tris, const int32_t* tri_link, int* nc,
+                             int* nloose, int32_t* ctri, int32_t* cnv, uint32_t* cvl, uint32_t* ctl, int32_t* loose);
 int ehr_render_mask_loss(ehr_ctx* ctx, const float* verts, const int32_t* tris, const int32_t* tri_link,
                          const int32_t* vert_link, const int32_t* opp, const float* mvp, const float* ref, int B,
                          int L, int V, int T, int H, int W, float* mask, float* loss, float* grad_mvp, void* stream);
```

Result: slower. 112,600 frames/s (-3.3%).
